# NVIDIA/tacotron2

Hardware: NVIDIA B200
Metric: mel frames/sec (B=64,T_text=150) (higher is better)
Workload: dtype f32 (split-fp16 tensor-core operands hi+lo, fp32 accumulate and state)

## Files before the change

### tacotron2_b200/_engine.py

```python
import contextlib
import ctypes as C
import threading

import torch

from . import _capi


def weight_table_spec(hp):
    E, K = hp.encoder_embedding_dim, hp.encoder_kernel_size
    s = [("embedding.weight", (hp.n_symbols, hp.symbols_embedding_dim))]

    def bn(p, c):
        return [(p + "weight", (c,)), (p + "bias", (c,)), (p + "running_mean", (c,)),
                (p + "running_var", (c,)), (p + "num_batches_tracked", ())]
    for i in range(hp.encoder_n_convolutions):
        p = "encoder.convolutions.%d." % i
        s += [(p + "0.conv.weight", (E, E, K)), (p + "0.conv.bias", (E,))] + bn(p + "1.", E)
    H = E // 2
    for suf in ("", "_reverse"):
        s += [("encoder.lstm.weight_ih_l0" + suf, (4 * H, E)), ("encoder.lstm.weight_hh_l0" + suf, (4 * H, H)),
              ("encoder.lstm.bias_ih_l0" + suf, (4 * H,)), ("encoder.lstm.bias_hh_l0" + suf, (4 * H,))]
    d = "decoder."
    nm = hp.n_mel_channels * hp.n_frames_per_step
    A, D, P = hp.attention_rnn_dim, hp.decoder_rnn_dim, hp.prenet_dim
    s += [(d + "prenet.layers.0.linear_layer.weight", (P, nm)), (d + "prenet.layers.1.linear_layer.weight", (P, P)),
          (d + "attention_rnn.weight_ih", (4 * A, P + E)), (d + "attention_rnn.weight_hh", (4 * A, A)),
          (d + "attention_rnn.bias_ih", (4 * A,)), (d + "attention_rnn.bias_hh", (4 * A,))]
    a = d + "attention_layer."
    s += [(a + "query_layer.linear_layer.weight", (hp.attention_dim, A)),
          (a + "memory_layer.linear_layer.weight", (hp.attention_dim, E)),
          (a + "v.linear_layer.weight", (1, hp.attention_dim)),
          (a + "location_layer.location_conv.conv.weight",
           (hp.attention_location_n_filters, 2, hp.attention_location_kernel_size)),
          (a + "location_layer.location_dense.linear_layer.weight", (hp.attention_dim, hp.attention_location_n_filters))]
    s += [(d + "decoder_rnn.weight_ih", (4 * D, A + E)), (d + "decoder_rnn.weight_hh", (4 * D, D)),
          (d + "decoder_rnn.bias_ih", (4 * D,)), (d + "decoder_rnn.bias_hh", (4 * D,)),
          (d + "linear_projection.linear_layer.weight", (nm, D + E)), (d + "linear_projection.linear_layer.bias", (nm,)),
          (d + "gate_layer.linear_layer.weight", (1, D + E)), (d + "gate_layer.linear_layer.bias", (1,))]
    PD, PK, n = hp.postnet_embedding_dim, hp.postnet_kernel_size, hp.postnet_n_convolutions
    for i in range(n):
        ci = hp.n_mel_channels if i == 0 else PD
        co = hp.n_mel_channels if i == n - 1 else PD
        p = "postnet.convolutions.%d." % i
        s += [(p + "0.conv.weight", (co, ci, PK)), (p + "0.conv.bias", (co,))] + bn(p + "1.", co)
    return s


_tls = threading.local()


@contextlib.contextmanager
def dropout_masks(prenet=None, att=None, dec=None, enc=None, post=None):
    prev = getattr(_tls, "masks", None)
    _tls.masks = dict(prenet=prenet, att=att, dec=dec, enc=enc, post=post)
    try:
        yield
    finally:
        _tls.masks = prev


def current_masks():
    return getattr(_tls, "masks", None) or dict(prenet=None, att=None, dec=None, enc=None, post=None)


_weights_generation = [0]


def bump_weights_generation():
    _weights_generation[0] += 1


def invalidate_weights():
    bump_weights_generation()


_seed_counter = [0]


def next_seed():
    _seed_counter[0] += 1
    return (torch.initial_seed() * 1000003 + _seed_counter[0]) & 0xFFFFFFFFFFFFFFFF


def _ptr(t):
    return C.c_void_p(t.data_ptr()) if t is not None else None


def _u8(mask, device):
    if mask is None:
        return None
    return mask.to(device=device, dtype=torch.uint8).contiguous()


class Engine:

    def __init__(self, hp):
        self.hp = hp
        self.spec = weight_table_spec(hp)
        self.handle = None
        self.key = None
        self.held = None
        self.device = None
        self._ws = {}
        self.impl = _capi.IMPL_AUTO

    def invalidate(self):
        self.key = None

    def ensure(self, named, force=False):
        dev = None
        for t in named.values():
            if t.is_cuda:
                dev = t.device
                break
        if dev is None:
            raise RuntimeError("tacotron2_b200: the model must live on a CUDA device (B200); there is no "
                               "CPU path -- call .cuda() first")
        key = (_weights_generation[0],) + tuple(
            (named[n].data_ptr(), named[n]._version, named[n].dtype) if n in named else None for n, _ in self.spec)
        if self.handle is not None and key == self.key and dev == self.device and not force:
            return
        L = _capi.lib()
        held, ptrs = [], (C.c_void_p * _capi.T2_NUM_WEIGHTS)()
        for i, (n, shape) in enumerate(self.spec):
            t = named.get(n)
            if n.endswith("num_batches_tracked"):
                ptrs[i] = None
                continue
            if t is None:
                t = torch.zeros(shape, device=dev, dtype=torch.float32)
                if n.endswith("running_var"):
                    t.fill_(1.0)
            else:
                if tuple(t.shape) != tuple(shape):
                    raise RuntimeError("tacotron2_b200: %s has shape %s, expected %s" % (n, tuple(t.shape), shape))
                t = t.detach()
                if t.dtype != torch.float32 or not t.is_contiguous():
                    t = t.float().contiguous()
            held.append(t)
            ptrs[i] = t.data_ptr()
        stream = C.c_void_p(torch.cuda.current_stream(dev).cuda_stream)
        with torch.cuda.device(dev):
            if self.handle is None or dev != self.device:
                self.close()
                hp = self.hp
                cfg = _capi.T2Config(
                    hp.n_mel_channels, hp.n_symbols, hp.symbols_embedding_dim, hp.encoder_kernel_size,
                    hp.encoder_n_convolutions, hp.encoder_embedding_dim, hp.attention_rnn_dim,
                    hp.decoder_rnn_dim, hp.prenet_dim, hp.attention_dim, hp.attention_location_n_filters,
                    hp.attention_location_kernel_size, hp.postnet_embedding_dim, hp.postnet_kernel_size,
                    hp.postnet_n_convolutions, hp.p_attention_dropout, hp.p_decoder_dropout, 1e-5)
                if hp.n_frames_per_step != 1:
                    raise RuntimeError("n_frames_per_step != 1 is not supported (hparams.py:56)")
                h = C.c_void_p()
                _capi.check(L.t2_model_create(C.byref(h), C.byref(cfg), ptrs, _capi.T2_NUM_WEIGHTS, stream))
                self.handle = h
            else:
                _capi.check(L.t2_model_refresh(self.handle, ptrs, _capi.T2_NUM_WEIGHTS, stream))
        self.key, self.held, self.device = key, held, dev

    def close(self):
        if self.handle is not None:
            _capi.lib().t2_model_destroy(self.handle)
            self.handle = None
            self.key = None

    def __del__(self):
        try:
            self.close()
        except Exception:
            pass

    def _workspace(self, tag, nbytes):
        t = self._ws.get(tag)
        if t is None or t.numel() < nbytes or t.device != self.device:
            t = torch.empty(int(nbytes), dtype=torch.uint8, device=self.device)
            self._ws[tag] = t
        return t

    def _stream(self):
        return C.c_void_p(torch.cuda.current_stream(self.device).cuda_stream)

    def encoder(self, text=None, embedded=None, lengths=None, training=False, keep=None, stash=None, seed=None):
        L = _capi.lib()
        src = text if text is not None else embedded
        B, T = int(src.shape[0]), int(src.shape[1])
        memory = torch.empty(B, T, self.hp.encoder_embedding_dim, device=self.device, dtype=torch.float32)
        ws = self._workspace("enc", L.t2_encoder_workspace_bytes(self.handle, B, T))
        a = _capi.T2EncoderArgs()
        if text is not None:
            text = text.to(device=self.device, dtype=torch.int64).contiguous()
            a.text = text.data_ptr()
        else:
            embedded = embedded.to(device=self.device, dtype=torch.float32).contiguous()
            a.embedded = embedded.data_ptr()
        len32 = None
        if lengths is not None:
            len32 = lengths.to(device=self.device, dtype=torch.int32).contiguous()
            a.lengths = len32.data_ptr()
        keep = _u8(keep, self.device)
        a.B, a.T, a.training = B, T, int(bool(training))
        a.keep = keep.data_ptr() if keep is not None else None
        a.seed = next_seed() if seed is None else seed
        a.memory, a.ws, a.ws_bytes = memory.data_ptr(), ws.data_ptr(), ws.numel()
        if stash is not None:
            a.stash, a.stash_bytes = stash.data_ptr(), stash.numel()
        with torch.cuda.device(self.device):
            _capi.check(L.t2_encoder_forward(self.handle, C.byref(a), self._stream()))
        return memory

    def stash_buffer(self, kind, *dims):
        n = getattr(_capi.lib(), "t2_%s_stash_bytes" % kind)(self.handle, *dims)
        return torch.empty(int(n), dtype=torch.uint8, device=self.device)

    def encoder_backward(self, text, embedded, lengths, training, keep, seed, stash, d_memory, want_d_embedded, named_grads):
        L = _capi.lib()
        B, T = int(d_memory.shape[0]), int(d_memory.shape[1])
        f32 = dict(device=self.device, dtype=torch.float32)
        a = _capi.T2EncoderBwdArgs()
        if text is not None:
            text = text.to(device=self.device, dtype=torch.int64).contiguous()
            a.text = text.data_ptr()
        else:
            embedded = embedded.to(**f32).contiguous()
            a.embedded = embedded.data_ptr()
        len32 = None
        if lengths is not None:
            len32 = lengths.to(device=self.device, dtype=torch.int32).contiguous()
            a.lengths = len32.data_ptr()
        keep = _u8(keep, self.device)
        a.B, a.T, a.training = B, T, int(bool(training))
        a.keep = keep.data_ptr() if keep is not None else None
        a.seed = seed
        a.stash, a.stash_bytes = stash.data_ptr(), stash.numel()
        d_memory = d_memory.to(**f32).contiguous()
        a.d_memory = d_memory.data_ptr()
        d_emb = torch.empty(B, T, self.hp.encoder_embedding_dim, **f32) if want_d_embedded else None
        a.d_embedded = d_emb.data_ptr() if d_emb is not None else None
        ptrs = self.grad_table(named_grads)
        a.grads, a.n_grads = ptrs, _capi.T2_NUM_WEIGHTS
        ws = self._workspace("enc_bwd", L.t2_encoder_backward_workspace_bytes(self.handle, B, T))
        a.ws, a.ws_bytes = ws.data_ptr(), ws.numel()
        with torch.cuda.device(self.device):
            _capi.check(L.t2_encoder_backward(self.handle, C.byref(a), self._stream()))
        return d_emb

    def postnet_backward(self, B, T, training, add_residual, keep, seed, stash, d_mel_post, named_grads, wgrad_lengths=None):
        L = _capi.lib()
        f32 = dict(device=self.device, dtype=torch.float32)
        a = _capi.T2PostnetBwdArgs()
        a.B, a.T, a.training, a.add_residual = B, T, int(bool(training)), int(bool(add_residual))
        if keep is not None and isinstance(keep, (list, tuple)):
            keep = torch.cat([k.to(torch.uint8).reshape(-1) for k in keep])
        keep = _u8(keep, self.device)
        a.keep = keep.data_ptr() if keep is not None else None
        a.seed = seed
        wl32 = None
        if wgrad_lengths is not None:
            wl32 = wgrad_lengths.to(device=self.device, dtype=torch.int32).contiguous()
            a.wgrad_lengths = wl32.data_ptr()
        a.stash, a.stash_bytes = stash.data_ptr(), stash.numel()
        d_mel_post = d_mel_post.to(**f32).contiguous()
        a.d_mel_post = d_mel_post.data_ptr()
        d_mel = torch.empty(B, T, self.hp.n_mel_channels, **f32)
        a.d_mel = d_mel.data_ptr()
        ptrs = self.grad_table(named_grads)
        a.grads, a.n_grads = ptrs, _capi.T2_NUM_WEIGHTS
        ws = self._workspace("post_bwd", L.t2_postnet_backward_workspace_bytes(self.handle, B, T))
        a.ws, a.ws_bytes = ws.data_ptr(), ws.numel()
        with torch.cuda.device(self.device):
            _capi.check(L.t2_postnet_backward(self.handle, C.byref(a), self._stream()))
        return d_mel

    def decoder(self, memory, mode, n_steps_cap, memory_lengths=None, teacher_prenet=None, training=False,
                prenet_keep=None, att_keep=None, dec_keep=None, gate_threshold=0.5,
                score_mask_value=-float("inf"), impl=None, stash=None, seed=None):
        L = _capi.lib()
        memory = memory.to(device=self.device, dtype=torch.float32).contiguous()
        B, T = int(memory.shape[0]), int(memory.shape[1])
        cap = int(n_steps_cap)
        mel = torch.zeros(B, cap, self.hp.n_mel_channels, device=self.device, dtype=torch.float32)
        gate = torch.zeros(B, cap, device=self.device, dtype=torch.float32)
        align = torch.zeros(B, cap, T, device=self.device, dtype=torch.float32)
        mel_lengths = torch.zeros(B, device=self.device, dtype=torch.int32)
        n_steps = torch.zeros(1, device=self.device, dtype=torch.int32)
        ws = self._workspace("dec", L.t2_decoder_workspace_bytes(self.handle, B, T, cap))
        a = _capi.T2DecoderArgs()
        a.mode, a.impl, a.training = mode, self.impl if impl is None else impl, int(bool(training))
        a.memory = memory.data_ptr()
        len32 = None
        if memory_lengths is not None:
            len32 = memory_lengths.to(device=self.device, dtype=torch.int32).contiguous()
            a.memory_lengths = len32.data_ptr()
        a.B, a.T_enc, a.n_steps_cap = B, T, cap
        if teacher_prenet is not None:
            teacher_prenet = teacher_prenet.contiguous()
            a.teacher_prenet = teacher_prenet.data_ptr()
        pk, ak, dk = _u8(prenet_keep, self.device), _u8(att_keep, self.device), _u8(dec_keep, self.device)
        a.prenet_keep = pk.data_ptr() if pk is not None else None
        a.att_keep = ak.data_ptr() if ak is not None else None
        a.dec_keep = dk.data_ptr() if dk is not None else None
        a.seed = next_seed() if seed is None else seed
        if stash is not None:
            a.stash, a.stash_bytes = stash.data_ptr(), stash.numel()
        a.gate_threshold = float(gate_threshold)
        a.score_mask_value = float(score_mask_value)
        a.mel, a.gate, a.align = mel.data_ptr(), gate.data_ptr(), align.data_ptr()
        a.mel_lengths, a.n_steps = mel_lengths.data_ptr(), n_steps.data_ptr()
        a.ws, a.ws_bytes = ws.data_ptr(), ws.numel()
        with torch.cuda.device(self.device):
            _capi.check(L.t2_decoder_run(self.handle, C.byref(a), self._stream()))
        self._last_decoder_args = (a, memory, len32, teacher_prenet, pk, ak, dk, ws, mel, gate, align, mel_lengths, n_steps)
        return mel, gate, align, mel_lengths, n_steps

    def decoder_profile(self):
        a = self._last_decoder_args[0]
        out = (C.c_int64 * 72)()
        _capi.check(_capi.lib().t2_decoder_profile(C.byref(a), out))
        names = ["E0 x2->att gemm", "E0 epilogue(ah)", "B1", "E1 ah->dec/att/q gemm", "B2", "attention", "B3",
                 "E2 ctx gemm", "E2 epilogue(dh)", "B4", "E3 dh gemm", "E3 epilogue(mel/x1)", "B5", "E4 x1 gemm+epi", "B6",
                 "att:im2col", "att:mma", "att:energies", "att:softmax", "att:context"]
        return {names[i]: [int(out[s * 24 + i]) for s in range(3)] for i in range(len(names))}

    def grad_table(self, named_grads):
        ptrs = (C.c_void_p * _capi.T2_NUM_WEIGHTS)()
        for i, (n, _) in enumerate(self.spec):
            t = named_grads.get(n)
            ptrs[i] = t.data_ptr() if t is not None else None
        return ptrs

    def decoder_stash(self, B, T_enc, T_mel):
        return self.stash_buffer("decoder", B, T_enc, T_mel)

    def decoder_backward(self, memory, memory_lengths, teacher_prenet, align, stash, seed, training, att_keep, dec_keep,
                         score_mask_value, d_mel, d_gate, d_align, named_grads):
        L = _capi.lib()
        B, Te = int(memory.shape[0]), int(memory.shape[1])
        T = int(align.shape[1])
        f32 = dict(device=self.device, dtype=torch.float32)
        d_memory = torch.empty(B, Te, self.hp.encoder_embedding_dim, **f32)
        d_prenet = torch.empty(T, B, self.hp.prenet_dim, **f32)
        ws = self._workspace("dec_bwd", L.t2_decoder_backward_workspace_bytes(self.handle, B, Te, T))
        a = _capi.T2DecoderBwdArgs()
        memory = memory.contiguous()
        a.memory = memory.data_ptr()
        len32 = None
        if memory_lengths is not None:
            len32 = memory_lengths.to(device=self.device, dtype=torch.int32).contiguous()
            a.memory_lengths = len32.data_ptr()
        a.B, a.T_enc, a.T_mel, a.training = B, Te, T, int(bool(training))
        a.teacher_prenet = teacher_prenet.data_ptr()
        ak, dk = _u8(att_keep, self.device), _u8(dec_keep, self.device)
        a.att_keep = ak.data_ptr() if ak is not None else None
        a.dec_keep = dk.data_ptr() if dk is not None else None
        a.seed, a.score_mask_value = seed, float(score_mask_value)
        a.align, a.stash, a.stash_bytes = align.data_ptr(), stash.data_ptr(), stash.numel()
        d_mel, d_gate = d_mel.to(**f32).contiguous(), d_gate.to(**f32).contiguous()
        a.d_mel, a.d_gate = d_mel.data_ptr(), d_gate.data_ptr()
        if d_align is not None:
            d_align = d_align.to(**f32).contiguous()
            a.d_align = d_align.data_ptr()
        a.d_memory, a.d_prenet = d_memory.data_ptr(), d_prenet.data_ptr()
        ptrs = self.grad_table(named_grads)
        a.grads, a.n_grads = ptrs, _capi.T2_NUM_WEIGHTS
        a.ws, a.ws_bytes = ws.data_ptr(), ws.numel()
        with torch.cuda.device(self.device):
            _capi.check(L.t2_decoder_backward(self.handle, C.byref(a), self._stream()))
        return d_memory, d_prenet

    def prenet_backward(self, frames, keep, seed, d_out, named_grads):
        L = _capi.lib()
        frames = frames.to(device=self.device, dtype=torch.float32).contiguous()
        M = int(frames.shape[0])
        d_out = d_out.contiguous()
        ws = self._workspace("pre_bwd", L.t2_prenet_backward_workspace_bytes(self.handle, M))
        keep = _u8(keep, self.device)
        a = _capi.T2PrenetBwdArgs()
        a.frames, a.M = frames.data_ptr(), M
        a.keep = keep.data_ptr() if keep is not None else None
        a.seed, a.d_out = seed, d_out.data_ptr()
        ptrs = self.grad_table(named_grads)
        a.grads, a.n_grads = ptrs, _capi.T2_NUM_WEIGHTS
        a.ws, a.ws_bytes = ws.data_ptr(), ws.numel()
        with torch.cuda.device(self.device):
            _capi.check(L.t2_prenet_backward(self.handle, C.byref(a), self._stream()))

    def prenet(self, frames, keep=None, seed=None):
        L = _capi.lib()
        frames = frames.to(device=self.device, dtype=torch.float32).contiguous()
        M = int(frames.shape[0])
        out = torch.empty(M, self.hp.prenet_dim, device=self.device, dtype=torch.float32)
        ws = self._workspace("pre", M * self.hp.prenet_dim * 4)
        keep = _u8(keep, self.device)
        with torch.cuda.device(self.device):
            _capi.check(L.t2_prenet_forward(self.handle, frames.data_ptr(), M,
                                            keep.data_ptr() if keep is not None else None,
                                            next_seed() if seed is None else seed,
                                            out.data_ptr(), ws.data_ptr(), ws.numel(), self._stream()))
        return out

    def postnet(self, mel_btc, lengths=None, add_residual=True, training=False, keep=None, stash=None, seed=None):
        L = _capi.lib()
        assert mel_btc.dtype == torch.float32 and mel_btc.stride(2) == 1 and mel_btc.stride(1) == mel_btc.shape[2]
        B, T = int(mel_btc.shape[0]), int(mel_btc.shape[1])
        out = torch.empty(B, self.hp.n_mel_channels, T, device=self.device, dtype=torch.float32)
        ws = self._workspace("post", L.t2_postnet_workspace_bytes(self.handle, B, T))
        a = _capi.T2PostnetArgs()
        a.mel, a.mel_batch_stride = mel_btc.data_ptr(), int(mel_btc.stride(0))
        len32 = None
        if lengths is not None:
            len32 = lengths.to(device=self.device, dtype=torch.int32).contiguous()
            a.lengths = len32.data_ptr()
        a.B, a.T, a.training = B, T, int(bool(training))
        if keep is not None and isinstance(keep, (list, tuple)):
            keep = torch.cat([k.to(torch.uint8).reshape(-1) for k in keep])
        keep = _u8(keep, self.device)
        a.keep = keep.data_ptr() if keep is not None else None
        a.seed = next_seed() if seed is None else seed
        a.add_residual = int(bool(add_residual))
        a.mel_post, a.ws, a.ws_bytes = out.data_ptr(), ws.data_ptr(), ws.numel()
        if stash is not None:
            a.stash, a.stash_bytes = stash.data_ptr(), stash.numel()
        with torch.cuda.device(self.device):
            _capi.check(L.t2_postnet_forward(self.handle, C.byref(a), self._stream()))
        return out

    def infer_host(self, text_host, max_steps, gate_threshold=0.5, impl=None, out_host=None):
        L = _capi.lib()
        B, T = int(text_host.shape[0]), int(text_host.shape[1])
        ws = self._workspace("e2e", L.t2_infer_workspace_bytes(self.handle, B, T, max_steps))
        if out_host is None:
            out_host = (torch.empty(B, self.hp.n_mel_channels, max_steps, dtype=torch.float32).pin_memory(),
                        torch.empty(B, dtype=torch.int32).pin_memory(), torch.empty(1, dtype=torch.int32).pin_memory())
        mel, lens, ns = out_host
        with torch.cuda.device(self.device):
            _capi.check(L.t2_infer_host(self.handle, text_host.data_ptr(), B, T, int(max_steps), float(gate_threshold),
                                        next_seed(), self.impl if impl is None else impl, mel.data_ptr(),
                                        lens.data_ptr(), ns.data_ptr(), ws.data_ptr(), ws.numel(), self._stream()))
        return mel, lens, ns
```

### tacotron2_b200/csrc/decoder.h

```cpp
#pragma once
#include "model.h"

namespace t2 {

constexpr int kMaxBatch = 1024;

struct DecoderCtrl {
  int all_done;
  int error;
  int pad_[2];
  unsigned int bar_count;
  unsigned int bar_gen;
  int pad2_[2];
  int done[kMaxBatch];
  long long prof[3][24];
  unsigned int x1_count; int pad3_[31];
  unsigned int x2_count; int pad4_[31];
  unsigned int ah_count[16]; int pad5_[16];
  unsigned int dh_count[16]; int pad6_[16];
};

struct DecoderWs {
  float* pm;
  char* state_begin; size_t state_bytes;
  float *ah, *ac, *dh, *dc;
  float* ctx;
  float *aw, *awc;
  float *x1, *x2;
  float* gates;
  float* proj;
  DecoderCtrl* ctrl;
  char* persistent; size_t persistent_bytes;
};

struct DecoderStash {
  float* ga = nullptr; float* gd = nullptr;
  float* ca = nullptr; float* ha = nullptr;
  float* cd = nullptr; float* hd = nullptr;
  float* ctx = nullptr;
};
inline size_t decoder_stash_bytes(int B, int T) {
  return ((size_t)2 * T * B * 4096 + (size_t)4 * (T + 1) * B * 1024 + (size_t)(T + 1) * B * 512) * sizeof(float);
}
inline void decoder_stash_carve(void* base, int B, int T, DecoderStash* s) {
  float* f = (float*)base;
  s->ga = f; f += (size_t)T * B * 4096;
  s->gd = f; f += (size_t)T * B * 4096;
  s->ca = f; f += (size_t)(T + 1) * B * 1024;
  s->ha = f; f += (size_t)(T + 1) * B * 1024;
  s->cd = f; f += (size_t)(T + 1) * B * 1024;
  s->hd = f; f += (size_t)(T + 1) * B * 1024;
  s->ctx = f;
}

size_t decoder_ws_bytes(int B, int T, int cap);
size_t persistent_ws_bytes(int B, int T, int cap);
int decoder_ws_carve(const T2DecoderArgs* a, DecoderWs* w);
int decoder_run_stepwise(T2Model* m, const T2DecoderArgs* a, cudaStream_t s);
int decoder_run_persistent(T2Model* m, const T2DecoderArgs* a, cudaStream_t s);
int decoder_backward(T2Model* m, const T2DecoderBwdArgs* a, cudaStream_t s);
size_t decoder_backward_ws_bytes(int B, int T_enc, int T_mel);
int prenet_backward(T2Model* m, const T2PrenetBwdArgs* a, cudaStream_t s);
bool persistent_supported(const T2Model* m, const T2DecoderArgs* a);

constexpr int kBwdGemmSplit = 4;
constexpr int kBwdImgBytes = 64 * 16384;
int bwd_gemm_prepare(T2Model* m, cudaStream_t s);
int bwd_gemm_run(T2Model* m, int which, const uint8_t* x_img, const float* inv_scale, float* P, int ldp, DecoderCtrl* ctrl,
                 cudaStream_t s);

}
```

### tacotron2_b200/csrc/decoder_persistent.cu

```cuda
#include <stdlib.h>
#include <string.h>

#include <vector>

#include "decoder.h"
#include "gemm_f32.cuh"
#include "umma.cuh"

namespace t2 {

namespace {

constexpr int kG = 128;
constexpr int kThreads = 512;
constexpr int kWarps = kThreads / 32;
constexpr int kStages = 4;
constexpr int kMaxStages = 5;
constexpr int kRows = 64;
constexpr int kXChunkBytes = 2 * kRows * kChunkK * 2;
constexpr int kColA = 0, kColD = 64, kColS = 128;
constexpr int kNA = 32, kND = 32, kNS = 16;
constexpr int kHiCols = 80;
constexpr int kColAtt = 160;
constexpr int kTmemCols = 512;
constexpr int kWStageMax = 2 * kHiCols * kChunkK * 2;
constexpr int kStageBytes = kXChunkBytes + kWStageMax;
constexpr int kNumEvents = 5;
constexpr int kPCols = 344;
constexpr int kQCta0 = 0, kQCtas = 16, kX2Cta0 = 16, kX2Ctas = 32, kPCta0 = 48, kPCtas = 43;
constexpr int kWeffBytes = kAtt * kChunkK * 2 * 2;
constexpr int kXchStride = 33;
constexpr unsigned long long kWatchdogCycles = 1ull << 32;

struct EventPlan {
  uint32_t w_off;
  uint32_t w_bytes;
  int32_t nrows;
  int32_t col0;
  int32_t ncons;
  int32_t n[3];
  int32_t chunks;
};
struct CtaPlan {
  EventPlan ev[kNumEvents];
};

struct BwdCta {
  EventPlan ep;
  int32_t chunk0, nchunks;
  int32_t col0, split;
};

struct PersistentPack {
  uint8_t* wimg = nullptr; size_t wimg_bytes = 0;
  CtaPlan* plans = nullptr;
  float* wp_all = nullptr;
  float* bias_p = nullptr;
  float* bias_a = nullptr;
  float* bias_d = nullptr;
  int32_t* rows = nullptr;
  float* weff = nullptr;
  uint8_t* weff_img = nullptr;
  uint8_t* bwd_wimg[2] = {nullptr, nullptr};
  struct BwdCta* bwd_plans[2] = {nullptr, nullptr};
};

__global__ void fuse_prenet_proj_kernel(const float* __restrict__ w1, const float* __restrict__ wp,
                                        const float* __restrict__ bp, float* __restrict__ out_w,
                                        float* __restrict__ out_b) {
  const int r = blockIdx.x;
  for (int c = threadIdx.x; c < kDRnn + kEnc; c += blockDim.x) {
    float s = 0.f;
    for (int k = 0; k < kMel; ++k) s = fmaf(w1[r * kMel + k], wp[(long)k * (kDRnn + kEnc) + c], s);
    out_w[(long)r * (kDRnn + kEnc) + c] = s;
  }
  if (threadIdx.x == 0) {
    float s = 0.f;
    for (int k = 0; k < kMel; ++k) s = fmaf(w1[r * kMel + k], bp[k], s);
    out_b[r] = s;
  }
}

__global__ void fuse_location_kernel(const float* __restrict__ wld, const float* __restrict__ wloc,
                                     float* __restrict__ weff) {
  const int d = blockIdx.x, kk = threadIdx.x;
  float s = 0.f;
  if (kk < 2 * kLocK) {
    const int ch = kk / kLocK, k = kk - ch * kLocK;
    for (int c = 0; c < kLocF; ++c) s = fmaf(wld[d * kLocF + c], wloc[(c * 2 + ch) * kLocK + k], s);
  }
  weff[d * kChunkK + kk] = s;
}

__global__ void pack_rows_image_kernel(const float* __restrict__ W, int N, int K, uint8_t* __restrict__ wimg) {
  const int chunk = blockIdx.x;
  __half* hi = reinterpret_cast<__half*>(wimg + (size_t)chunk * N * 256);
  __half* lo = hi + N * 64;
  for (int i = threadIdx.x; i < N * 64; i += blockDim.x) {
    const int r = i >> 6, k = i & 63;
    __half h, l;
    split_fp16(W[(long)r * K + chunk * 64 + k], h, l);
    const uint32_t e = img_elem_offset(r, k);
    hi[e] = h; lo[e] = l;
  }
}

__global__ void pack_consumer_kernel(const float* __restrict__ src, int ld, int kcol0,
                                     const int32_t* __restrict__ rows_tab, const CtaPlan* __restrict__ plans,
                                     int ev, int cons, uint8_t* __restrict__ wimg) {
  const int cta = blockIdx.y, chunk = blockIdx.x;
  const EventPlan& ep = plans[cta].ev[ev];
  if (cons >= ep.ncons) return;
  const int n = ep.n[cons];
  int roff = 0;
  for (int i = 0; i < cons; ++i) roff += 2 * ep.n[i];
  __half* img = reinterpret_cast<__half*>(wimg + ep.w_off + (size_t)chunk * ep.w_bytes);
  for (int i = threadIdx.x; i < n * 64; i += blockDim.x) {
    const int r = i >> 6, k = i & 63;
    const int srow = rows_tab[cta * 32 + r];
    const float v = srow >= 0 ? src[(long)srow * ld + kcol0 + chunk * 64 + k] : 0.f;
    __half h, l;
    split_fp16(v, h, l);
    img[img_elem_offset(roff + r, k)] = h;
    img[img_elem_offset(roff + n + r, k)] = l;
  }
}

__global__ void pack_lstm_bias_kernel(const float* __restrict__ b_sum, float* __restrict__ out) {
  const int i = blockIdx.x * blockDim.x + threadIdx.x;
  if (i >= kG * 32) return;
  const int cta = i >> 5, col = i & 31, ul = col >> 2, g = col & 3;
  out[i] = b_sum[g * 1024 + cta * 8 + ul];
}

__global__ void rows_to_image_kernel(const float* __restrict__ src, long ld, int n_rows, int K,
                                     long src_block_stride, uint8_t* __restrict__ dst, long dst_block_stride) {
  const float* s = src + (long)blockIdx.y * src_block_stride;
  uint8_t* d = dst + (long)blockIdx.y * dst_block_stride;
  const int chunk = blockIdx.x;
  __half* hi = reinterpret_cast<__half*>(d + (long)chunk * kXChunkBytes);
  __half* lo = hi + kRows * kChunkK;
  for (int i = threadIdx.x; i < kRows * kChunkK; i += blockDim.x) {
    const int r = i >> 6, k = i & 63;
    const int kk = chunk * kChunkK + k;
    const float v = (r < n_rows && kk < K) ? s[(long)r * ld + kk] : 0.f;
    __half h, l;
    split_fp16(v, h, l);
    const uint32_t e = img_elem_offset(r, k);
    hi[e] = h; lo[e] = l;
  }
}

__device__ __forceinline__ void watchdog_trap(DecoderCtrl* ctrl, int code) {
  if (ctrl) ctrl->error = code;
  __threadfence_system();
  __trap();
}

__device__ __forceinline__ void mbar_wait(uint64_t* bar, uint32_t parity, DecoderCtrl* ctrl, int code) {
  if (ptx::mbar_try_wait(bar, parity)) return;
  const unsigned long long t0 = clock64();
  while (!ptx::mbar_try_wait(bar, parity)) {
    if (clock64() - t0 > kWatchdogCycles) watchdog_trap(ctrl, code);
  }
}

__device__ __forceinline__ void arrive_release(unsigned int* cnt) {
  asm volatile("fence.acq_rel.gpu;" ::: "memory");
  asm volatile("red.relaxed.gpu.global.add.u32 [%0], 1;" ::"l"(cnt) : "memory");
}
__device__ __forceinline__ void poll_acquire(unsigned int* cnt, unsigned int target, DecoderCtrl* ctrl, int code) {
  const unsigned long long t0 = clock64();
  while (true) {
    unsigned int c;
    asm volatile("ld.relaxed.gpu.global.u32 %0, [%1];" : "=r"(c) : "l"(cnt) : "memory");
    if ((int)(c - target) >= 0) break;
    if (clock64() - t0 > kWatchdogCycles) watchdog_trap(ctrl, code);
  }
  asm volatile("fence.acq_rel.gpu;" ::: "memory");
}

__device__ __forceinline__ void grid_barrier(DecoderCtrl* ctrl, unsigned int& target, uint32_t cs, uint32_t rank) {
  ptx::fence_proxy_async();
  if (cs > 1) {
    __threadfence();
    ptx::cluster_sync_all();
    target += gridDim.x / cs;
    if (rank == 0 && threadIdx.x == 0) {
      asm volatile("red.release.gpu.global.add.u32 [%0], 1;" ::"l"(&ctrl->bar_count) : "memory");
      const unsigned long long t0 = clock64();
      while (true) {
        unsigned int c;
        asm volatile("ld.acquire.gpu.global.u32 %0, [%1];" : "=r"(c) : "l"(&ctrl->bar_count) : "memory");
        if ((int)(c - target) >= 0) break;
        if (clock64() - t0 > kWatchdogCycles) watchdog_trap(ctrl, 100);
      }
      __threadfence();
    }
    ptx::cluster_sync_all();
    ptx::fence_proxy_async();
    return;
  }
  __syncthreads();
  target += gridDim.x;
  if (threadIdx.x == 0) {
    arrive_release(&ctrl->bar_count);
    poll_acquire(&ctrl->bar_count, target, ctrl, 100);
  }
  __syncthreads();
  ptx::fence_proxy_async();
}

__device__ __forceinline__ void grid_arrive(DecoderCtrl* ctrl, unsigned int& target) {
  ptx::fence_proxy_async();
  __syncthreads();
  target += gridDim.x;
  if (threadIdx.x == 0) {
    arrive_release(&ctrl->bar_count);
  }
}
__device__ __forceinline__ void grid_wait(DecoderCtrl* ctrl, unsigned int target) {
  if (threadIdx.x == 0) {
    poll_acquire(&ctrl->bar_count, target, ctrl, 101);
  }
  __syncthreads();
  ptx::fence_proxy_async();
}

constexpr unsigned int kStopFlag = 1u << 24;
__device__ __forceinline__ void signal_counter(unsigned int* cnt, unsigned int inc) {
  ptx::fence_proxy_async();
  __syncthreads();
  if (threadIdx.x == 0) {
    asm volatile("fence.acq_rel.gpu;" ::: "memory");
    asm volatile("red.relaxed.gpu.global.add.u32 [%0], %1;" ::"l"(cnt), "r"(inc) : "memory");
  }
}
__device__ __forceinline__ bool wait_counter(unsigned int* cnt, unsigned int target, int* s_flag, DecoderCtrl* ctrl, int code) {
  if (threadIdx.x == 0) {
    const unsigned long long t0 = clock64();
    unsigned int c;
    while (true) {
      asm volatile("ld.relaxed.gpu.global.u32 %0, [%1];" : "=r"(c) : "l"(cnt) : "memory");
      if ((c & (kStopFlag - 1u)) >= target) break;
      if (clock64() - t0 > kWatchdogCycles) watchdog_trap(ctrl, code);
    }
    asm volatile("fence.acq_rel.gpu;" ::: "memory");
    *s_flag = (int)(c >> 24);
  }
  __syncthreads();
  ptx::fence_proxy_async();
  return *s_flag != 0;
}

__device__ __forceinline__ float sigmoid_exact(float x) { return 1.f / (1.f + expf(-x)); }
__device__ __forceinline__ float sigmoid_fast(float x) { return __fdividef(1.f, 1.f + __expf(-x)); }
__device__ __forceinline__ float tanh_fast(float x) { return 2.f * sigmoid_fast(2.f * x) - 1.f; }
__device__ __forceinline__ float warp_sum_f(float v) {
#pragma unroll
  for (int o = 16; o > 0; o >>= 1) v += __shfl_xor_sync(0xffffffffu, v, o);
  return v;
}
__device__ __forceinline__ float warp_max_f(float v) {
#pragma unroll
  for (int o = 16; o > 0; o >>= 1) v = fmaxf(v, __shfl_xor_sync(0xffffffffu, v, o));
  return v;
}

struct Ring {
  uint8_t* stage0;
  __device__ __forceinline__ uint8_t* stage(uint32_t s) const { return stage0 + s * kStageBytes; }
  uint64_t* full;
  uint64_t* empty;
  uint64_t* acc;
  uint32_t p_stage, p_phase;
  uint32_t c_stage, c_phase;
  uint32_t acc_phase;
  uint64_t pol_x, pol_w;
  uint32_t cs, rank;
  uint32_t pre;
  uint32_t ns;
};

__device__ __forceinline__ void prefetch_weights(Ring& rg, const EventPlan& nx, const uint8_t* w_img,
                                                 DecoderCtrl* ctrl) {
  uint32_t s = rg.p_stage, ph = rg.p_phase;
  const uint32_t n = min(rg.ns, (uint32_t)nx.chunks);
  for (uint32_t i = 0; i < n; ++i) {
    mbar_wait(&rg.empty[s], ph ^ 1, ctrl, 205);
    ptx::mbar_arrive_expect_tx(&rg.full[s], kXChunkBytes + nx.w_bytes);
    ptx::bulk_g2s_hint(rg.stage(s) + kXChunkBytes, w_img + nx.w_off + (size_t)i * nx.w_bytes, nx.w_bytes,
                       &rg.full[s], rg.pol_w);
    if (++s == rg.ns) { s = 0; ph ^= 1; }
  }
  rg.pre = n;
}

__device__ __forceinline__ void run_event(Ring& rg, const EventPlan& ep, const uint8_t* x_img,
                                          const uint8_t* w_img, int chunks, uint32_t tmem_base,
                                          DecoderCtrl* ctrl, const EventPlan* next,
                                          const unsigned int* ready = nullptr, unsigned int ready_target = 0) {
  const int warp = threadIdx.x >> 5, lane = threadIdx.x & 31;
  if (ep.nrows == 0) {
    if (threadIdx.x == 0 && next != nullptr && next->nrows != 0 && rg.pre == 0) prefetch_weights(rg, *next, w_img, ctrl);
    return;
  }
  if (warp == 0) {
    if (lane == 0) {
      int nready = ready ? 0 : chunks;
      for (int i = 0; i < chunks; ++i) {
        uint8_t* st = rg.stage(rg.p_stage);
        if ((uint32_t)i >= rg.pre) {
          mbar_wait(&rg.empty[rg.p_stage], rg.p_phase ^ 1, ctrl, 200);
          ptx::mbar_arrive_expect_tx(&rg.full[rg.p_stage], kXChunkBytes + ep.w_bytes);
          ptx::bulk_g2s_hint(st + kXChunkBytes, w_img + ep.w_off + (size_t)i * ep.w_bytes, ep.w_bytes,
                             &rg.full[rg.p_stage], rg.pol_w);
        }
        if (i >= nready) {
          const unsigned long long t0 = clock64();
          while (true) {
            uint32_t c[16];
#pragma unroll
            for (int j = 0; j < 16; j += 4)
              asm volatile("ld.relaxed.gpu.global.v4.u32 {%0,%1,%2,%3}, [%4];"
                           : "=r"(c[j]), "=r"(c[j + 1]), "=r"(c[j + 2]), "=r"(c[j + 3]) : "l"(ready + j) : "memory");
            uint32_t mask = 0;
#pragma unroll
            for (int j = 0; j < 16; ++j) mask |= ((int)(c[j] - ready_target) >= 0 ? 1u : 0u) << j;
            const int run = __ffs((int)~(mask >> i)) - 1;
            if (run > 0) { nready = min(chunks, i + run); break; }
            if (clock64() - t0 > kWatchdogCycles) watchdog_trap(ctrl, 206);
          }
          asm volatile("fence.acq_rel.gpu;" ::: "memory");
          ptx::fence_proxy_async();
        }
        if (rg.cs == 1) {
          ptx::bulk_g2s_hint(st, x_img + (size_t)i * kXChunkBytes, kXChunkBytes, &rg.full[rg.p_stage], rg.pol_x);
        } else {
          const uint32_t slice = kXChunkBytes / rg.cs;
          ptx::bulk_g2s_mc_hint(st + rg.rank * slice, x_img + (size_t)i * kXChunkBytes + rg.rank * slice, slice,
                                &rg.full[rg.p_stage], (uint16_t)((1u << rg.cs) - 1u), rg.pol_x);
        }
        if (++rg.p_stage == rg.ns) { rg.p_stage = 0; rg.p_phase ^= 1; }
      }
      rg.pre = 0;
      if (next != nullptr && next->nrows != 0) prefetch_weights(rg, *next, w_img, ctrl);
    }
    __syncwarp();
  } else if (warp == 1) {
    if (lane == 0) {
      const uint32_t idesc = ptx::make_idesc_f16(128, 2u * (uint32_t)ep.nrows);
      const uint32_t d = tmem_base + (uint32_t)ep.col0;
      for (int i = 0; i < chunks; ++i) {
        mbar_wait(&rg.full[rg.c_stage], rg.c_phase, ctrl, 201);
        ptx::tc_fence_after();
        const uint32_t xs = ptx::smem_u32(rg.stage(rg.c_stage));
        const uint32_t ws = xs + kXChunkBytes;
#pragma unroll
        for (int kk = 0; kk < kChunkK / 16; ++kk) {
          const uint64_t a = ptx::make_sw128_desc(xs + kk * 32);
          const uint64_t b = ptx::make_sw128_desc(ws + kk * 32);
          ptx::umma_f16(d, a, b, idesc, 1u);
        }
        if (rg.cs == 1) ptx::umma_commit(&rg.empty[rg.c_stage]);
        else ptx::umma_commit_mc(&rg.empty[rg.c_stage], (uint16_t)((1u << rg.cs) - 1u));
        if (++rg.c_stage == rg.ns) { rg.c_stage = 0; rg.c_phase ^= 1; }
      }
      ptx::umma_commit(rg.acc);
    }
    __syncwarp();
  }
  mbar_wait(rg.acc, rg.acc_phase, ctrl, 202);
  rg.acc_phase ^= 1;
  ptx::tc_fence_after();
}

__device__ __forceinline__ uint32_t philox_keep8(uint64_t seed, uint32_t site, uint64_t idx0, float pdrop) {
  uint32_t bits = 0;
  uint64_t blk_cur = ~0ull;
  uint32_t o[4] = {0, 0, 0, 0};
#pragma unroll
  for (int i = 0; i < 8; ++i) {
    const uint64_t idx = idx0 + i, blk = idx >> 2;
    if (blk != blk_cur) {
      philox4x32_10((uint32_t)blk, (uint32_t)(blk >> 32), site, 0x7ac07201u, (uint32_t)seed, (uint32_t)(seed >> 32), o);
      blk_cur = blk;
    }
    const float u = (float)(o[idx & 3] >> 8) * (1.0f / 16777216.0f);
    bits |= (u >= pdrop ? 1u : 0u) << i;
  }
  return bits;
}

__device__ __forceinline__ void acc_take8(uint32_t t_lane, int base, int n, int col, float* s) {
  float a[8], b[8];
  ptx::tmem_ld8(t_lane + base + col, a);
  ptx::tmem_ld8(t_lane + base + n + col, b);
#pragma unroll
  for (int i = 0; i < 8; ++i) s[i] = a[i] + b[i];
  ptx::tmem_zero8(t_lane + base + col);
  ptx::tmem_zero8(t_lane + base + n + col);
  ptx::tmem_wait_st();
}

__device__ __forceinline__ void stash_lstm(float* gates, float* cs, float* hs, int t, int Btot, int b, int unit0,
                                           const float (&sg)[4][2], const float (&c)[2], const float (&h)[2]) {
  float* gp = gates + ((long)t * Btot + b) * (4 * kARnn) + unit0;
#pragma unroll
  for (int g = 0; g < 4; ++g) *reinterpret_cast<float2*>(gp + g * kARnn) = make_float2(sg[g][0], sg[g][1]);
  const long o = ((long)(t + 1) * Btot + b) * kARnn + unit0;
  *reinterpret_cast<float2*>(cs + o) = make_float2(c[0], c[1]);
  *reinterpret_cast<float2*>(hs + o) = make_float2(h[0], h[1]);
}

struct KParams {
  const CtaPlan* plans;
  const uint8_t* wimg;
  const float* bias_a; const float* bias_d; const float* bias_p;
  const uint8_t* weff_img; const float* w_v;
  float l2_pin_frac;
  const float* memory; const float* pm; const int32_t* mem_len;
  const uint8_t* prenet_keep; const uint8_t* att_keep; const uint8_t* dec_keep;
  uint8_t* x2_img; uint8_t* ah_img; uint8_t* ctx_img; uint8_t* dh_img; uint8_t* x1_img;
  const uint8_t* teacher_x2_img;
  float* q;
  float* mel; float* gate; float* align; int32_t* mel_lengths; int32_t* n_steps;
  DecoderCtrl* ctrl;
  int B, T, cap, infer, training, cluster, hier_barrier;
  int nstages;
  int chunk_ready;
  int b0, Btot;
  float gate_threshold, score_mask_value, p_att, p_dec;
  uint64_t seed;
  DecoderStash st;
};

__device__ __forceinline__ void store_split2(uint8_t* img, int row, int k, float v0, float v1) {
  const int chunk = k >> 6, kc = k & 63;
  __half h0, l0, h1, l1;
  split_fp16(v0, h0, l0);
  split_fp16(v1, h1, l1);
  __half* hi = reinterpret_cast<__half*>(img + (size_t)chunk * kXChunkBytes);
  __half* lo = hi + kRows * kChunkK;
  const uint32_t e = img_elem_offset(row, kc);
  *reinterpret_cast<__half2*>(hi + e) = __halves2half2(h0, h1);
  *reinterpret_cast<__half2*>(lo + e) = __halves2half2(l0, l1);
}

__global__ void __launch_bounds__(kThreads, 1) decoder_persistent_kernel(const KParams p) {
  extern __shared__ __align__(1024) uint8_t smem_raw[];
  const int tid = threadIdx.x, warp = tid >> 5, lane = tid & 31;
  const int cta = blockIdx.x;
  const int T = p.T, TP = T + kLocK - 1;
  const int ntiles = (T + 127) >> 7;

  uint8_t* sp = smem_raw;
  Ring rg;
  rg.ns = (uint32_t)p.nstages;
  rg.stage0 = sp; sp += p.nstages * kStageBytes;
  uint8_t* s_weff = sp; sp += kWeffBytes;
  uint64_t* bars = reinterpret_cast<uint64_t*>(sp); sp += 16 * sizeof(uint64_t);
  rg.full = bars; rg.empty = bars + kMaxStages; rg.acc = bars + 2 * kMaxStages;
  uint32_t* tmem_slot = reinterpret_cast<uint32_t*>(sp); sp += 16;
  int* s_live = reinterpret_cast<int*>(sp); sp += 16;
  int* s_flag = s_live + 1;
  float* s_bias_a = reinterpret_cast<float*>(sp); sp += 32 * 4;
  float* s_bias_d = reinterpret_cast<float*>(sp); sp += 32 * 4;
  float* s_v = reinterpret_cast<float*>(sp); sp += kAtt * 4;
  float* s_q = reinterpret_cast<float*>(sp); sp += kAtt * 4;
  float* s_red = reinterpret_cast<float*>(sp); sp += 32 * 4;
  uint32_t* s_mask = reinterpret_cast<uint32_t*>(sp); sp += kRows * 4;
  float* s_bias_p = reinterpret_cast<float*>(sp); sp += 8 * 4;
  long long* s_prof = reinterpret_cast<long long*>(sp); sp += 24 * 8;
  float* s_pad0 = reinterpret_cast<float*>(sp); sp += ((TP + 3) & ~3) * 4;
  float* s_pad1 = reinterpret_cast<float*>(sp); sp += ((TP + 3) & ~3) * 4;
  float* s_xch = reinterpret_cast<float*>(sp);
  float* s_e = reinterpret_cast<float*>(sp);
  float* s_ep = s_e + ntiles * 128;
  (void)s_red;

  rg.p_stage = rg.p_phase = rg.c_stage = rg.c_phase = rg.acc_phase = 0;
  rg.cs = p.cluster; rg.rank = p.cluster > 1 ? ptx::cluster_ctarank() : 0;
  rg.pre = 0;

  if (tid == 0) {
    for (int s = 0; s < p.nstages; ++s) { ptx::mbar_init(&rg.full[s], 1); ptx::mbar_init(&rg.empty[s], rg.cs); }
    ptx::mbar_init(rg.acc, 1);
    ptx::fence_barrier_init();
  }
  if (warp == 2) ptx::tmem_alloc<kTmemCols>(tmem_slot);
  for (int i = tid; i < 32; i += kThreads) { s_bias_a[i] = p.bias_a[cta * 32 + i]; s_bias_d[i] = p.bias_d[cta * 32 + i]; }
  for (int i = tid; i < kWeffBytes / 16; i += kThreads)
    reinterpret_cast<uint4*>(s_weff)[i] = reinterpret_cast<const uint4*>(p.weff_img)[i];
  {
    uint64_t pol;
    asm volatile("createpolicy.fractional.L2::evict_last.L2::evict_first.b64 %0, %1;" : "=l"(pol) : "f"(p.l2_pin_frac));
    rg.pol_w = pol;
    rg.pol_x = ptx::policy_evict_last();
  }
  for (int i = tid; i < kAtt; i += kThreads) s_v[i] = p.w_v[i];
  if (tid < 8) s_bias_p[tid] = (cta >= kPCta0 && cta < kPCta0 + kPCtas) ? p.bias_p[(cta - kPCta0) * 8 + tid] : 0.f;
  for (int i = tid; i < TP; i += kThreads) { s_pad0[i] = 0.f; s_pad1[i] = 0.f; }
  ptx::fence_proxy_async();
  ptx::tc_fence_before();
  __syncthreads();
  if (p.cluster > 1) ptx::cluster_sync_all();
  ptx::tc_fence_after();
  const uint32_t tmem_base = *tmem_slot;

  const CtaPlan& plan = p.plans[cta];
  DecoderCtrl* ctrl = p.ctrl;
  unsigned int bar_target = 0;
  const uint32_t bar_cs = p.hier_barrier ? rg.cs : 1;
  const int quad = warp & 3, cg = warp >> 2;
  const int row = (quad & 1) * 32 + lane;
  const bool is_lo = quad >= 2;
  const bool erow = !is_lo && row < p.B;
  const uint32_t t_lane = tmem_base + ((uint32_t)(quad * 32) << 16);
  float c_att[2] = {0.f, 0.f}, c_dec[2] = {0.f, 0.f};
  const bool has_q = cta >= kQCta0 && cta < kQCta0 + kQCtas;
  const bool has_x2 = cta >= kX2Cta0 && cta < kX2Cta0 + kX2Ctas;
  const bool has_p = cta >= kPCta0 && cta < kPCta0 + kPCtas;
  const int halfk = (kLocK - 1) / 2;
  for (int c = cg * 40; c < cg * 40 + 40; c += 8) ptx::tmem_zero8(t_lane + c);
  ptx::tmem_wait_st();
  ptx::tc_fence_before();
  __syncthreads();
  const int prof_slot = cta == 0 ? 0 : (cta == 60 ? 1 : (cta == 100 ? 2 : -1));
  long long prof_last = clock64();
  if (tid < 24) s_prof[tid] = 0;
#define T2_PROF(ph)                                                        \
  do {                                                                     \
    if (prof_slot >= 0 && tid == 0) {                                      \
      const long long now_ = clock64();                                    \
      s_prof[ph] += now_ - prof_last;    \
      prof_last = now_;                                                    \
    }                                                                      \
  } while (0)
#define T2_TAKE_GATES(colbase, n_, g)                                                        \
  do {                                                                                   \
    acc_take8(t_lane, (colbase), (n_), cg * 8, g);                                       \
    if (is_lo) {                                                                         \
      _Pragma("unroll") for (int i_ = 0; i_ < 8; ++i_) s_xch[row * kXchStride + cg * 8 + i_] = g[i_]; \
    }                                                                                    \
    ptx::tc_fence_before();                                                              \
    __syncthreads();                                                                     \
    if (!is_lo) {                                                                        \
      _Pragma("unroll") for (int i_ = 0; i_ < 8; ++i_) g[i_] += s_xch[row * kXchStride + cg * 8 + i_]; \
    }                                                                                    \
  } while (0)

  auto x2_epilogue = [&]() {
    float g[8];
    if (cg == 0) acc_take8(t_lane, kColS, kNS, 0, g);
    if (cg == 0 && is_lo) {
#pragma unroll
      for (int i = 0; i < 8; ++i) s_xch[row * kXchStride + i] = g[i];
    }
    ptx::tc_fence_before();
    __syncthreads();
    if (cg == 0 && erow) {
      const int col0 = (cta - kX2Cta0) * 8;
      float r[8];
      const uint32_t bits = s_mask[row];
#pragma unroll
      for (int j = 0; j < 8; ++j)
        r[j] = ((bits >> j) & 1u) ? fmaxf(g[j] + s_xch[row * kXchStride + j], 0.f) * 2.f : 0.f;
#pragma unroll
      for (int j = 0; j < 8; j += 2) store_split2(p.x2_img, row, col0 + j, r[j], r[j + 1]);
    }
  };

  int t = 0;
  for (; t < p.cap; ++t) {
    {
      const uint8_t* x2 = p.infer ? p.x2_img : p.teacher_x2_img + (size_t)t * 4 * kXChunkBytes;
      run_event(rg, plan.ev[0], x2, p.wimg, 4, tmem_base, ctrl, &plan.ev[1]);
      T2_PROF(0);
      float g[8];
      T2_TAKE_GATES(kColA, kNA, g);
      if (erow) {
        float hv[2], sg[4][2];
#pragma unroll
        for (int u = 0; u < 2; ++u) {
          const float* b = s_bias_a + (cg * 2 + u) * 4;
          const float gi = sigmoid_fast(g[u * 4 + 0] + b[0]);
          const float gf = sigmoid_fast(g[u * 4 + 1] + b[1]);
          const float gg = tanh_fast(g[u * 4 + 2] + b[2]);
          const float go = sigmoid_fast(g[u * 4 + 3] + b[3]);
          c_att[u] = gf * c_att[u] + gi * gg;
          float h = go * tanh_fast(c_att[u]);
          if (p.training) {
            const int unit = cta * 8 + cg * 2 + u;
            const long idx = (long)(p.b0 + row) * kARnn + unit;
            const bool keep = p.att_keep ? p.att_keep[(long)t * p.Btot * kARnn + idx] != 0
                                         : philox_keep(p.seed, t * 4 + 2, idx, p.p_att);
            h = keep ? h * (1.f / (1.f - p.p_att)) : 0.f;
          }
          hv[u] = h;
          sg[0][u] = gi; sg[1][u] = gf; sg[2][u] = gg; sg[3][u] = go;
        }
        store_split2(p.ah_img, row, cta * 8 + cg * 2, hv[0], hv[1]);
        if (p.st.ga) stash_lstm(p.st.ga, p.st.ca, p.st.ha, t, p.Btot, p.b0 + row, cta * 8 + cg * 2, sg, c_att, hv);
      }
      T2_PROF(1);
      if (p.chunk_ready) signal_counter(&ctrl->ah_count[cta >> 3], 1u);
      else grid_barrier(ctrl, bar_target, bar_cs, rg.rank);
      T2_PROF(2);
    }
    {
      if (p.infer && is_lo && cg == 0 && row < p.B && t + 1 < p.cap && (has_p || has_x2)) {
        uint32_t bits = 0;
        if (has_x2) {
          const int col0 = (cta - kX2Cta0) * 8;
          if (p.prenet_keep) {
            const uint8_t* kp = p.prenet_keep + ((long)(t + 1) * 2 + 1) * p.Btot * kPre + (long)(p.b0 + row) * kPre + col0;
            for (int j = 0; j < 8; ++j) bits |= (kp[j] != 0 ? 1u : 0u) << j;
          } else {
            bits = philox_keep8(p.seed, (t + 1) * 4 + 1, (uint64_t)(p.b0 + row) * kPre + col0, 0.5f);
          }
        } else {
          const int pc0 = (cta - kPCta0) * 8;
          for (int j = 0; j < 8; ++j) {
            const int col = pc0 + j - (kMel + 1);
            if (col < 0 || col >= kPre) continue;
            const long idx = (long)(p.b0 + row) * kPre + col;
            const bool keep = p.prenet_keep ? p.prenet_keep[((long)(t + 1) * 2 + 0) * p.Btot * kPre + idx] != 0
                                            : philox_keep(p.seed, (t + 1) * 4 + 0, idx, 0.5f);
            bits |= (keep ? 1u : 0u) << j;
          }
        }
        s_mask[row] = bits;
      }
      run_event(rg, plan.ev[1], p.ah_img, p.wimg, 16, tmem_base, ctrl, nullptr,
                p.chunk_ready ? ctrl->ah_count : nullptr, 8u * (unsigned int)(t + 1));
      if (has_q) {
        float g[8];
        if (cg == 0) acc_take8(t_lane, kColS, kNS, 0, g);
        if (cg == 0 && is_lo) {
#pragma unroll
          for (int i = 0; i < 8; ++i) s_xch[row * kXchStride + i] = g[i];
        }
        ptx::tc_fence_before();
        __syncthreads();
        if (cg == 0 && erow) {
#pragma unroll
          for (int j = 0; j < 8; ++j) p.q[row * kAtt + (cta - kQCta0) * 8 + j] = g[j] + s_xch[row * kXchStride + j];
        }
      }
      T2_PROF(3);
    }
    const bool att_cta = (cta & 63) < p.B;
    const int att_b = cta & 63, ahalf = cta >> 6;
    uint8_t* aimg = rg.stage0;
    const int att_rounds = (T + 255) >> 8;
    const int img_plane = att_rounds > 1 ? 32768 : max(4096, ((T + 15) & ~15) * 128);
    const int img_bytes = 2 * img_plane;
    const int smem_rows = min(T, (p.nstages * kStageBytes - img_bytes) / (kEnc / 2 * 4));
    auto att_im2col_mma_tr = [&](int r0) {
      const int jbase = r0 * 256, cnt = min(T - jbase, 256), npad = (cnt + 15) & ~15;
      for (int item = tid; item < npad * 8; item += kThreads) {
        const int jj = item >> 3, g8 = item & 7, j = jbase + jj;
        __align__(16) __half hh[8];
        __align__(16) __half ll[8];
#pragma unroll
        for (int e = 0; e < 8; ++e) {
          const int kk = g8 * 8 + e;
          float v = 0.f;
          if (jj < cnt && kk < 2 * kLocK) v = kk < kLocK ? s_pad0[j + kk] : s_pad1[j + kk - kLocK];
          split_fp16(v, hh[e], ll[e]);
        }
        uint8_t* dst = aimg + (jj >> 3) * 1024 + (jj & 7) * 128 + ((g8 ^ (jj & 7)) * 16);
        *reinterpret_cast<uint4*>(dst) = *reinterpret_cast<const uint4*>(hh);
        *reinterpret_cast<uint4*>(dst + img_plane) = *reinterpret_cast<const uint4*>(ll);
      }
      ptx::fence_proxy_async();
      __syncthreads();
      if (warp == 1) {
        if (lane == 0) {
          ptx::tc_fence_after();
          const uint32_t ws = ptx::smem_u32(s_weff), ps = ptx::smem_u32(aimg);
          const uint32_t idesc = ptx::make_idesc_f16(128, (uint32_t)npad);
          const uint32_t d = tmem_base + kColAtt;
#pragma unroll
          for (int kk = 0; kk < kChunkK / 16; ++kk) {
            const uint64_t w_hi = ptx::make_sw128_desc(ws + kk * 32);
            const uint64_t w_lo = ptx::make_sw128_desc(ws + 16384 + kk * 32);
            const uint64_t p_hi = ptx::make_sw128_desc(ps + kk * 32);
            const uint64_t p_lo = ptx::make_sw128_desc(ps + (uint32_t)img_plane + kk * 32);
            ptx::umma_f16(d, w_hi, p_hi, idesc, kk > 0 ? 1u : 0u);
            ptx::umma_f16(d, w_lo, p_hi, idesc, 1u);
            ptx::umma_f16(d, w_hi, p_lo, idesc, 1u);
          }
          ptx::umma_commit(rg.acc);
        }
        __syncwarp();
      }
    };
    auto stage_memory_rows = [&](int j0, int j1) {
      const uint32_t sbase = ptx::smem_u32(rg.stage0) + (uint32_t)img_bytes;
      const float* msrc = p.memory + (long)att_b * T * kEnc + ahalf * (kEnc / 2);
      for (int i = j0 * 64 + tid; i < j1 * 64; i += kThreads) {
        const int j = i >> 6, c4 = i & 63;
        asm volatile("cp.async.cg.shared.global [%0], [%1], 16;" ::"r"(sbase + (uint32_t)i * 16u),
                     "l"(msrc + (long)j * kEnc + c4 * 4)
                     : "memory");
      }
      asm volatile("cp.async.commit_group;" ::: "memory");
    };
    grid_arrive(ctrl, bar_target);
    const int adim = quad * 32 + lane;
    float pm_next[8];
    auto load_pm = [&](const float* pmr, int j0, int cnt) {
#pragma unroll
      for (int e = 0; e < 8; ++e) pm_next[e] = (j0 + e < cnt) ? __ldg(pmr + (long)(j0 + e) * kAtt) : 0.f;
    };
    if (att_cta) {
      att_im2col_mma_tr(0);
      stage_memory_rows(0, smem_rows);
      load_pm(p.pm + (long)att_b * T * kAtt + adim, cg * 8, min(T, 256));
    }
    T2_PROF(15);
    grid_wait(ctrl, bar_target);
    T2_PROF(4);
    if (att_cta) {
      const int b = att_b;
      for (int i = tid; i < kAtt; i += kThreads) s_q[i] = __ldcg(&p.q[b * kAtt + i]);
      __syncthreads();
      {
        const int eN = ntiles * 128;
        const float qd = s_q[adim], vd = s_v[adim];
        const int nrounds = att_rounds;
        for (int r0 = 0; r0 < nrounds; ++r0) {
          const int jbase = r0 * 256, cnt = min(T - jbase, 256), nch = (((cnt + 15) & ~15) >> 3);
          if (r0 > 0) att_im2col_mma_tr(r0);
          mbar_wait(rg.acc, rg.acc_phase, ctrl, 203);
          rg.acc_phase ^= 1;
          ptx::tc_fence_after();
          T2_PROF(16);
          const float* pmr = p.pm + ((long)b * T + jbase) * kAtt + adim;
          if (r0 > 0) load_pm(pmr, cg * 8, cnt);
#pragma unroll 1
          for (int c = cg; c < nch; c += 4) {
            const int j0 = c * 8;
            float pm8[8];
#pragma unroll
            for (int e = 0; e < 8; ++e) pm8[e] = pm_next[e];
            if (c + 4 < nch) load_pm(pmr, j0 + 32, cnt);
            float g[8], sv[8];
            ptx::tmem_ld8(t_lane + kColAtt + j0, g);
#pragma unroll
            for (int e = 0; e < 8; ++e) sv[e] = vd * tanh_fast(qd + g[e] + pm8[e]);
            float r4[4], r2[2], r1;
            {
              const bool up = (lane & 16) != 0;
#pragma unroll
              for (int e = 0; e < 4; ++e) {
                const float send = up ? sv[e] : sv[e + 4], keep = up ? sv[e + 4] : sv[e];
                r4[e] = keep + __shfl_xor_sync(0xffffffffu, send, 16);
              }
            }
            {
              const bool up = (lane & 8) != 0;
#pragma unroll
              for (int e = 0; e < 2; ++e) {
                const float send = up ? r4[e] : r4[e + 2], keep = up ? r4[e + 2] : r4[e];
                r2[e] = keep + __shfl_xor_sync(0xffffffffu, send, 8);
              }
            }
            {
              const bool up = (lane & 4) != 0;
              const float send = up ? r2[0] : r2[1], keep = up ? r2[1] : r2[0];
              r1 = keep + __shfl_xor_sync(0xffffffffu, send, 4);
            }
            r1 += __shfl_xor_sync(0xffffffffu, r1, 2);
            r1 += __shfl_xor_sync(0xffffffffu, r1, 1);
            const int jj = j0 + ((lane >> 4) & 1) * 4 + ((lane >> 3) & 1) * 2 + ((lane >> 2) & 1);
            if ((lane & 3) == 0 && jj < cnt) s_ep[quad * eN + jbase + jj] = r1;
          }
          ptx::tc_fence_before();
          __syncthreads();
          T2_PROF(17);
        }
      }
      const int len = p.mem_len ? p.mem_len[b] : T;
      const int eN = ntiles * 128;
      for (int j = tid; j < T; j += kThreads)
        s_ep[j] = (j < len) ? (s_ep[j] + s_ep[eN + j]) + (s_ep[2 * eN + j] + s_ep[3 * eN + j]) : p.score_mask_value;
      __syncthreads();
      float mx = -INFINITY;
      for (int j = lane; j < T; j += 32) mx = fmaxf(mx, s_ep[j]);
      mx = warp_max_f(mx);
      float sum = 0.f;
      for (int j = lane; j < T; j += 32) sum += expf(s_ep[j] - mx);
      sum = warp_sum_f(sum);
      const float inv = 1.f / sum;
      for (int j = tid; j < T; j += kThreads) {
        const float a = expf(s_ep[j] - mx) * inv;
        s_e[j] = a;
        s_pad0[halfk + j] = a;
        s_pad1[halfk + j] += a;
        if (ahalf == 0) p.align[((long)b * p.cap + t) * T + j] = a;
      }
      asm volatile("cp.async.wait_group 0;" ::: "memory");
      __syncthreads();
      T2_PROF(18);
      {
        const int c4 = tid & 63, jg = tid >> 6;
        const float4* ms = reinterpret_cast<const float4*>(rg.stage0 + img_bytes);
        float4 acc = make_float4(0.f, 0.f, 0.f, 0.f);
#pragma unroll 4
        for (int j = jg; j < smem_rows; j += 8) {
          const float4 m = ms[j * 64 + c4];
          const float a = s_e[j];
          acc.x = fmaf(a, m.x, acc.x); acc.y = fmaf(a, m.y, acc.y); acc.z = fmaf(a, m.z, acc.z); acc.w = fmaf(a, m.w, acc.w);
        }
        const float* mp = p.memory + (long)b * T * kEnc + ahalf * (kEnc / 2) + c4 * 4;
        for (int j = smem_rows + jg; j < T; j += 8) {
          const float4 m = __ldg(reinterpret_cast<const float4*>(mp + (long)j * kEnc));
          const float a = s_e[j];
          acc.x = fmaf(a, m.x, acc.x); acc.y = fmaf(a, m.y, acc.y); acc.z = fmaf(a, m.z, acc.z); acc.w = fmaf(a, m.w, acc.w);
        }
        __syncthreads();
        float* scr = reinterpret_cast<float*>(rg.stage0);
        *reinterpret_cast<float4*>(scr + jg * (kEnc / 2) + c4 * 4) = acc;
        __syncthreads();
        if (tid < kEnc / 4) {
          const int col = tid * 2;
          float v0 = 0.f, v1 = 0.f;
#pragma unroll
          for (int g = 0; g < 8; ++g) { v0 += scr[g * (kEnc / 2) + col]; v1 += scr[g * (kEnc / 2) + col + 1]; }
          store_split2(p.ctx_img, b, ahalf * (kEnc / 2) + col, v0, v1);
          if (p.st.ga)
            *reinterpret_cast<float2*>(p.st.ctx + ((long)(t + 1) * p.Btot + p.b0 + b) * kEnc + ahalf * (kEnc / 2) + col) =
                make_float2(v0, v1);
        }
      }
      T2_PROF(19);
    }
    T2_PROF(5);
    grid_barrier(ctrl, bar_target, bar_cs, rg.rank);
    T2_PROF(6);
    {
      run_event(rg, plan.ev[2], p.ctx_img, p.wimg, 8, tmem_base, ctrl, &plan.ev[3]);
      T2_PROF(7);
      float g[8];
      T2_TAKE_GATES(kColD, kND, g);
      if (erow) {
        float hv[2], sg[4][2];
#pragma unroll
        for (int u = 0; u < 2; ++u) {
          const float* b = s_bias_d + (cg * 2 + u) * 4;
          const float gi = sigmoid_fast(g[u * 4 + 0] + b[0]);
          const float gf = sigmoid_fast(g[u * 4 + 1] + b[1]);
          const float gg = tanh_fast(g[u * 4 + 2] + b[2]);
          const float go = sigmoid_fast(g[u * 4 + 3] + b[3]);
          c_dec[u] = gf * c_dec[u] + gi * gg;
          float h = go * tanh_fast(c_dec[u]);
          if (p.training) {
            const int unit = cta * 8 + cg * 2 + u;
            const long idx = (long)(p.b0 + row) * kDRnn + unit;
            const bool keep = p.dec_keep ? p.dec_keep[(long)t * p.Btot * kDRnn + idx] != 0
                                         : philox_keep(p.seed, t * 4 + 3, idx, p.p_dec);
            h = keep ? h * (1.f / (1.f - p.p_dec)) : 0.f;
          }
          hv[u] = h;
          sg[0][u] = gi; sg[1][u] = gf; sg[2][u] = gg; sg[3][u] = go;
        }
        store_split2(p.dh_img, row, cta * 8 + cg * 2, hv[0], hv[1]);
        if (p.st.ga) stash_lstm(p.st.gd, p.st.cd, p.st.hd, t, p.Btot, p.b0 + row, cta * 8 + cg * 2, sg, c_dec, hv);
      }
      T2_PROF(8);
      if (p.chunk_ready) signal_counter(&ctrl->dh_count[cta >> 3], 1u);
      else grid_barrier(ctrl, bar_target, bar_cs, rg.rank);
      T2_PROF(9);
    }
    {
      run_event(rg, plan.ev[3], p.dh_img, p.wimg, 16, tmem_base, ctrl,
                (!p.infer && t + 1 < p.cap) ? &plan.ev[0] : nullptr,
                p.chunk_ready ? ctrl->dh_count : nullptr, 8u * (unsigned int)(t + 1));
      T2_PROF(10);
      if (tid == 0) *s_live = 0;
      float g[8];
      if (has_p && cg == 0) acc_take8(t_lane, kColS, kNS, 0, g);
      if (has_p && cg == 0 && is_lo) {
#pragma unroll
        for (int i = 0; i < 8; ++i) s_xch[row * kXchStride + i] = g[i];
      }
      ptx::tc_fence_before();
      __syncthreads();
      if (has_p && cg == 0 && erow) {
        const int pc0 = (cta - kPCta0) * 8;
#pragma unroll
        for (int j = 0; j < 8; ++j) {
          const int pc = pc0 + j;
          const float v = g[j] + s_xch[row * kXchStride + j] + s_bias_p[j];
          if (pc < kMel) {
            p.mel[((long)row * p.cap + t) * kMel + pc] = v;
          } else if (pc == kMel) {
            p.gate[(long)row * p.cap + t] = v;
            if (p.infer) {
              int done = ctrl->done[row];
              if (!done && sigmoid_exact(v) > p.gate_threshold) {
                done = 1; ctrl->done[row] = 1; p.mel_lengths[row] = t + 1;
              }
              if (!done) atomicAdd(s_live, 1);
            }
          } else if (pc < kMel + 1 + kPre) {
            const int col = pc - (kMel + 1);
            float r = fmaxf(v, 0.f);
            if (p.infer && t + 1 < p.cap) r = ((s_mask[row] >> j) & 1u) ? r * 2.f : 0.f;
            if (p.infer) {
              __half h, l;
              split_fp16(r, h, l);
              __half* hi = reinterpret_cast<__half*>(p.x1_img + (size_t)(col >> 6) * kXChunkBytes);
              __half* lo = hi + kRows * kChunkK;
              const uint32_t e = img_elem_offset(row, col & 63);
              hi[e] = h; lo[e] = l;
            }
          }
        }
      }
      __syncthreads();
      const bool gate_cta = has_p && (cta - kPCta0) * 8 <= kMel && (cta - kPCta0) * 8 + 8 > kMel;
      if (gate_cta && tid == 0) atomicMax(p.n_steps, t + 1);
      T2_PROF(11);
      if (!p.infer) continue;
      bool stop = t + 1 == p.cap;
      if (has_p) signal_counter(&ctrl->x1_count, 1u + ((gate_cta && *s_live == 0) ? kStopFlag : 0u));
      if (has_x2) {
        stop |= wait_counter(&ctrl->x1_count, (unsigned int)(kPCtas * (t + 1)), s_flag, ctrl, 102);
        if (!stop) {
          run_event(rg, plan.ev[4], p.x1_img, p.wimg, 4, tmem_base, ctrl, nullptr);
          x2_epilogue();
        }
        signal_counter(&ctrl->x2_count, 1u + (stop ? kStopFlag : 0u));
      }
      T2_PROF(12);
      stop |= wait_counter(&ctrl->x2_count, (unsigned int)(kX2Ctas * (t + 1)), s_flag, ctrl, 103);
      T2_PROF(14);
      if (stop) { ++t; break; }
    }
  }
  if (prof_slot >= 0 && tid == 0)
    for (int i = 0; i < 24; ++i) ctrl->prof[prof_slot][i] = s_prof[i];
  if (cta == 0) {
    __syncthreads();
    const int ns = p.infer ? t : p.cap;
    for (int b = tid; b < p.B; b += kThreads)
      if (!p.infer || !__ldcg(&ctrl->done[b])) p.mel_lengths[b] = ns;
    if (tid == 0) atomicMax(p.n_steps, ns);
  }
  if (p.cluster > 1) {
    if (tid == 0)
      for (int s = 0; s < p.nstages; ++s) {
        mbar_wait(&rg.empty[rg.p_stage], rg.p_phase ^ 1, ctrl, 204);
        if (++rg.p_stage == rg.ns) { rg.p_stage = 0; rg.p_phase ^= 1; }
      }
    __syncthreads();
    ptx::cluster_sync_all();
  }
  ptx::tc_fence_before();
  __syncthreads();
  if (warp == 2) ptx::tmem_dealloc<kTmemCols>(tmem_base);
}

}

static size_t persistent_smem_bytes(int T, int nstages) {
  const int TP = T + kLocK - 1;
  const int ntiles = (T + 127) / 128;
  const size_t xch = (size_t)kRows * kXchStride * 4, att = (size_t)5 * ntiles * 128 * 4;
  return (size_t)nstages * kStageBytes + kWeffBytes + 16 * 8 + 16 + 16 + 2 * 32 * 4 + kAtt * 4 + kAtt * 4 + 32 * 4 +
         kRows * 4 + 32 + 24 * 8 + 2 * (size_t)((TP + 3) & ~3) * 4 + (xch > att ? xch : att) + 1024;
}
constexpr size_t kSmemLimit = 227 * 1024;
static int persistent_stages(int T) {
  int want = 4;
  const char* e = getenv("T2_STAGES");
  if (e && atoi(e) >= 3 && atoi(e) <= kMaxStages) want = atoi(e);
  while (want > 4 && persistent_smem_bytes(T, want) > kSmemLimit) --want;
  return want;
}

size_t persistent_ws_bytes(int B, int T, int cap) {
  (void)B; (void)T;
  return (size_t)(4 + 16 + 8 + 16 + 4) * kXChunkBytes + (size_t)kRows * kAtt * 4 + 1024 +
         (size_t)cap * 4 * kXChunkBytes;
}

bool persistent_supported(const T2Model* m, const T2DecoderArgs* a) {
  if (!m->pk) return false;
  if (m->sm_count < kG) return false;
  if (persistent_smem_bytes(a->T_enc, 4) > kSmemLimit) return false;
  return true;
}

int persistent_pack_create(T2Model* m, cudaStream_t s) {
  PersistentPack* pk = (PersistentPack*)m->pk;
  if (!pk) { pk = new PersistentPack(); m->pk = pk; }
  const int kdc = kDRnn + kEnc;
  std::vector<CtaPlan> plans(kG);
  size_t off = 0;
  for (int c = 0; c < kG; ++c) {
    const bool hq = c >= kQCta0 && c < kQCta0 + kQCtas, hx = c >= kX2Cta0 && c < kX2Cta0 + kX2Ctas,
               hp = c >= kPCta0 && c < kPCta0 + kPCtas;
    CtaPlan& pl = plans[c];
    memset(&pl, 0, sizeof(pl));
    auto set = [&](int ev, int chunks, int col0, std::initializer_list<int> ns) {
      EventPlan& e = pl.ev[ev];
      e.ncons = 0; e.nrows = 0; e.col0 = col0;
      for (int n : ns) { e.n[e.ncons++] = n; e.nrows += n; }
      e.w_bytes = (uint32_t)e.nrows * 256;
      e.w_off = (uint32_t)off;
      e.chunks = chunks;
      off += (size_t)chunks * e.w_bytes;
    };
    set(0, 4, kColA, {32});
    if (hq) set(1, 16, kColA, {32, 32, 16}); else set(1, 16, kColA, {32, 32});
    if (hp) set(2, 8, kColA, {32, 32, 16}); else set(2, 8, kColA, {32, 32});
    if (hp) set(3, 16, kColD, {32, 16}); else set(3, 16, kColD, {32});
    if (hx) set(4, 4, kColS, {16}); else { pl.ev[4].w_off = (uint32_t)off; }
  }
  if (off >= (size_t)4 << 30) return fail(T2_ERR_INVALID, "W image too large");
  if (!pk->wimg) {
    pk->wimg_bytes = off + 1024;
    T2_CUDA(cudaMalloc((void**)&pk->wimg, pk->wimg_bytes));
    T2_CUDA(cudaMalloc((void**)&pk->plans, sizeof(CtaPlan) * kG));
    T2_CUDA(cudaMalloc((void**)&pk->wp_all, (size_t)kPCols * kdc * 4));
    T2_CUDA(cudaMalloc((void**)&pk->bias_p, (size_t)kPCols * 4));
    T2_CUDA(cudaMalloc((void**)&pk->bias_a, (size_t)kG * 32 * 4));
    T2_CUDA(cudaMalloc((void**)&pk->bias_d, (size_t)kG * 32 * 4));
    T2_CUDA(cudaMalloc((void**)&pk->rows, (size_t)4 * kG * 32 * 4));
    T2_CUDA(cudaMalloc((void**)&pk->weff, (size_t)kAtt * kChunkK * 4));
    T2_CUDA(cudaMalloc((void**)&pk->weff_img, (size_t)kWeffBytes));
  }
  fuse_location_kernel<<<kAtt, kChunkK, 0, s>>>(m->w[W_ATT_LOC_DENSE], m->w[W_ATT_LOC_CONV], pk->weff);
  T2_LAUNCH_CHECK();
  pack_rows_image_kernel<<<1, 256, 0, s>>>(pk->weff, kAtt, kChunkK, pk->weff_img);
  T2_LAUNCH_CHECK();
  T2_CUDA(cudaMemcpyAsync(pk->plans, plans.data(), sizeof(CtaPlan) * kG, cudaMemcpyHostToDevice, s));
  T2_CUDA(cudaStreamSynchronize(s));
  T2_CUDA(cudaMemsetAsync(pk->wp_all, 0, (size_t)kPCols * kdc * 4, s));
  T2_CUDA(cudaMemsetAsync(pk->bias_p, 0, (size_t)kPCols * 4, s));
  T2_CUDA(cudaMemcpyAsync(pk->wp_all, m->projgate_w, (size_t)(kMel + 1) * kdc * 4, cudaMemcpyDeviceToDevice, s));
  T2_CUDA(cudaMemcpyAsync(pk->bias_p, m->projgate_b, (size_t)(kMel + 1) * 4, cudaMemcpyDeviceToDevice, s));
  fuse_prenet_proj_kernel<<<kPre, 256, 0, s>>>(m->w[W_PRENET0], m->w[W_PROJ_W], m->w[W_PROJ_B],
                                               pk->wp_all + (size_t)(kMel + 1) * kdc, pk->bias_p + kMel + 1);
  T2_LAUNCH_CHECK();
  pack_lstm_bias_kernel<<<(kG * 32 + 255) / 256, 256, 0, s>>>(m->arnn_b, pk->bias_a);
  T2_LAUNCH_CHECK();
  pack_lstm_bias_kernel<<<(kG * 32 + 255) / 256, 256, 0, s>>>(m->drnn_b, pk->bias_d);
  T2_LAUNCH_CHECK();
  std::vector<int32_t> rows((size_t)4 * kG * 32, -1);
  for (int c = 0; c < kG; ++c) {
    for (int col = 0; col < 32; ++col) rows[(0 * kG + c) * 32 + col] = (col & 3) * 1024 + c * 8 + (col >> 2);
    if (c >= kQCta0 && c < kQCta0 + kQCtas) for (int j = 0; j < 8; ++j) rows[(1 * kG + c) * 32 + j] = (c - kQCta0) * 8 + j;
    if (c >= kPCta0 && c < kPCta0 + kPCtas) for (int j = 0; j < 8; ++j) rows[(2 * kG + c) * 32 + j] = (c - kPCta0) * 8 + j;
    if (c >= kX2Cta0 && c < kX2Cta0 + kX2Ctas) for (int j = 0; j < 8; ++j) rows[(3 * kG + c) * 32 + j] = (c - kX2Cta0) * 8 + j;
  }
  T2_CUDA(cudaMemcpyAsync(pk->rows, rows.data(), rows.size() * 4, cudaMemcpyHostToDevice, s));
  T2_CUDA(cudaStreamSynchronize(s));
  const int32_t* r_lstm = pk->rows; const int32_t* r_q = pk->rows + kG * 32;
  const int32_t* r_p = pk->rows + 2 * kG * 32; const int32_t* r_x2 = pk->rows + 3 * kG * 32;
  auto pack = [&](const float* src, int ld, int kcol0, int chunks, const int32_t* rt, int ev, int cons) -> int {
    pack_consumer_kernel<<<dim3(chunks, kG), 256, 0, s>>>(src, ld, kcol0, rt, pk->plans, ev, cons, pk->wimg);
    T2_LAUNCH_CHECK();
    return T2_OK;
  };
  T2_TRY(pack(m->w[W_ARNN_WIH], kPre + kEnc, 0, 4, r_lstm, 0, 0));
  T2_TRY(pack(m->w[W_ARNN_WHH], kARnn, 0, 16, r_lstm, 1, 0));
  T2_TRY(pack(m->w[W_DRNN_WIH], kdc, 0, 16, r_lstm, 1, 1));
  T2_TRY(pack(m->w[W_ATT_QUERY], kARnn, 0, 16, r_q, 1, 2));
  T2_TRY(pack(m->w[W_ARNN_WIH], kPre + kEnc, kPre, 8, r_lstm, 2, 0));
  T2_TRY(pack(m->w[W_DRNN_WIH], kdc, kARnn, 8, r_lstm, 2, 1));
  T2_TRY(pack(pk->wp_all, kdc, kDRnn, 8, r_p, 2, 2));
  T2_TRY(pack(m->w[W_DRNN_WHH], kDRnn, 0, 16, r_lstm, 3, 0));
  T2_TRY(pack(pk->wp_all, kdc, 0, 16, r_p, 3, 1));
  T2_TRY(pack(m->w[W_PRENET1], kPre, 0, 4, r_x2, 4, 0));
  return T2_OK;
}

void persistent_pack_destroy(T2Model* m) {
  PersistentPack* pk = (PersistentPack*)m->pk;
  if (!pk) return;
  cudaFree(pk->wimg); cudaFree(pk->plans); cudaFree(pk->wp_all); cudaFree(pk->bias_p);
  cudaFree(pk->bias_a); cudaFree(pk->bias_d); cudaFree(pk->rows); cudaFree(pk->weff); cudaFree(pk->weff_img);
  for (int i = 0; i < 2; ++i) { cudaFree(pk->bwd_wimg[i]); cudaFree(pk->bwd_plans[i]); }
  delete pk;
  m->pk = nullptr;
}

static int run_persistent_slice(T2Model* m, const T2DecoderArgs* a, cudaStream_t s, int b0, int nb);

int decoder_run_persistent(T2Model* m, const T2DecoderArgs* a, cudaStream_t s) {
  T2_CUDA(cudaMemsetAsync(a->n_steps, 0, sizeof(int32_t), s));
  for (int b0 = 0; b0 < a->B; b0 += kRows) {
    const int nb = a->B - b0 < kRows ? a->B - b0 : kRows;
    T2_TRY(run_persistent_slice(m, a, s, b0, nb));
  }
  return T2_OK;
}

static int run_persistent_slice(T2Model* m, const T2DecoderArgs* a, cudaStream_t s, int b0, int nb) {
  PersistentPack* pk = (PersistentPack*)m->pk;
  const int B = nb, T = a->T_enc, cap = a->n_steps_cap;
  DecoderWs w;
  T2_TRY(decoder_ws_carve(a, &w));
  T2_CUDA(cudaMemsetAsync(w.ctrl, 0, sizeof(DecoderCtrl), s));
  T2_CUDA(cudaMemsetAsync(w.persistent, 0, (size_t)(4 + 16 + 8 + 16 + 4) * kXChunkBytes + (size_t)kRows * kAtt * 4, s));
  {
    GemmArgs g;
    g.seg[0] = {a->memory + (size_t)b0 * T * kEnc, kEnc, m->w[W_ATT_MEMORY], kEnc, kEnc};
    g.M = B * T; g.N = kAtt; g.C = w.pm; g.ldc = kAtt;
    T2_TRY(gemm_f32(g, s));
  }
  KParams p;
  memset(&p, 0, sizeof(p));
  uint8_t* img = (uint8_t*)w.persistent;
  p.x2_img = img; img += 4 * kXChunkBytes;
  p.ah_img = img; img += 16 * kXChunkBytes;
  p.ctx_img = img; img += 8 * kXChunkBytes;
  p.dh_img = img; img += 16 * kXChunkBytes;
  p.x1_img = img; img += 4 * kXChunkBytes;
  p.q = (float*)img;
  p.plans = pk->plans; p.wimg = pk->wimg; p.bias_a = pk->bias_a; p.bias_d = pk->bias_d; p.bias_p = pk->bias_p;
  p.weff_img = pk->weff_img; p.w_v = m->w[W_ATT_V];
  {
    const char* e = getenv("T2_L2_PIN_FRAC");
    p.l2_pin_frac = e ? (float)atof(e) : 0.5f;
  }
  p.memory = a->memory + (size_t)b0 * T * kEnc; p.pm = w.pm;
  p.mem_len = a->memory_lengths ? a->memory_lengths + b0 : nullptr;
  p.prenet_keep = a->prenet_keep; p.att_keep = a->att_keep; p.dec_keep = a->dec_keep;
  p.mel = a->mel + (size_t)b0 * cap * kMel; p.gate = a->gate + (size_t)b0 * cap; p.align = a->align + (size_t)b0 * cap * T;
  p.mel_lengths = a->mel_lengths + b0; p.n_steps = a->n_steps;
  p.ctrl = w.ctrl;
  p.b0 = b0; p.Btot = a->B;
  p.B = B; p.T = T; p.cap = cap; p.infer = a->mode == T2_MODE_INFER; p.training = a->training;
  p.gate_threshold = a->gate_threshold; p.score_mask_value = a->score_mask_value;
  p.p_att = m->cfg.p_attention_dropout; p.p_dec = m->cfg.p_decoder_dropout; p.seed = a->seed;
  if (a->stash) {
    if (p.infer) return fail(T2_ERR_INVALID, "the training stash needs T2_MODE_TEACHER");
    if (a->stash_bytes < decoder_stash_bytes(a->B, cap)) return fail(T2_ERR_WORKSPACE, "decoder stash too small");
    decoder_stash_carve(a->stash, a->B, cap, &p.st);
    if (b0 == 0) {
      float* z[5] = {p.st.ca, p.st.ha, p.st.cd, p.st.hd, p.st.ctx};
      for (int i = 0; i < 5; ++i)
        T2_CUDA(cudaMemsetAsync(z[i], 0, (size_t)a->B * (i < 4 ? kARnn : kEnc) * sizeof(float), s));
    }
  }
  if (!p.infer) {
    uint8_t* timg = (uint8_t*)p.q + (size_t)kRows * kAtt * 4;
    timg = (uint8_t*)(((uintptr_t)timg + 1023) & ~(uintptr_t)1023);
    rows_to_image_kernel<<<dim3(4, cap), 256, 0, s>>>(a->teacher_prenet + (size_t)b0 * kPre, kPre, B, kPre, (long)a->B * kPre, timg,
                                                      (long)4 * kXChunkBytes);
    T2_LAUNCH_CHECK();
    p.teacher_x2_img = timg;
  }
  p.nstages = persistent_stages(T);
  {
  }
  {
    const char* e = getenv("T2_CHUNK_READY");
    p.chunk_ready = (e && !strcmp(e, "0")) ? 0 : 1;
  }
  const size_t smem = persistent_smem_bytes(T, p.nstages);
  T2_CUDA(cudaFuncSetAttribute(decoder_persistent_kernel, cudaFuncAttributeMaxDynamicSharedMemorySize, (int)smem));
  T2_CUDA(cudaFuncSetAttribute(decoder_persistent_kernel, cudaFuncAttributeNonPortableClusterSizeAllowed, 1));
  int want = 1;
  {
    const char* e = getenv("T2_CLUSTER");
    if (e) want = atoi(e);
    if (want != 1 && want != 2 && want != 4 && want != 8) want = 1;
  }
  {
    p.hier_barrier = 0;
  }
  cudaLaunchConfig_t cfg;
  memset(&cfg, 0, sizeof(cfg));
  cfg.gridDim = dim3(kG); cfg.blockDim = dim3(kThreads); cfg.dynamicSmemBytes = smem; cfg.stream = s;
  cudaLaunchAttribute attrs[2];
  for (p.cluster = want; p.cluster > 1; p.cluster >>= 1) {
    attrs[0].id = cudaLaunchAttributeClusterDimension;
    attrs[0].val.clusterDim.x = p.cluster; attrs[0].val.clusterDim.y = 1; attrs[0].val.clusterDim.z = 1;
    cfg.attrs = attrs; cfg.numAttrs = 1;
    int max_clusters = 0;
    if (cudaOccupancyMaxActiveClusters(&max_clusters, decoder_persistent_kernel, &cfg) == cudaSuccess &&
        max_clusters * p.cluster >= kG)
      break;
    (void)cudaGetLastError();
  }
  int na = 0;
  if (p.cluster > 1) {
    attrs[na].id = cudaLaunchAttributeClusterDimension;
    attrs[na].val.clusterDim.x = p.cluster; attrs[na].val.clusterDim.y = 1; attrs[na].val.clusterDim.z = 1; ++na;
  }
  attrs[na].id = cudaLaunchAttributeCooperative; attrs[na].val.cooperative = 1; ++na;
  cfg.attrs = attrs; cfg.numAttrs = na;
  cudaError_t le = cudaLaunchKernelEx(&cfg, decoder_persistent_kernel, p);
  if (le != cudaSuccess && p.cluster > 1) {
    (void)cudaGetLastError();
    cfg.numAttrs = 1;
    le = cudaLaunchKernelEx(&cfg, decoder_persistent_kernel, p);
  }
  if (le != cudaSuccess) return fail(T2_ERR_CUDA, "persistent decoder launch failed: %s", cudaGetErrorString(le));
  if (getenv("T2_VERBOSE")) fprintf(stderr, "[t2b200] persistent decoder: B=%d T_enc=%d cap=%d cluster=%d stages=%d chunk_ready=%d smem=%zu\n",
                                    B, T, cap, p.cluster, p.nstages, p.chunk_ready, smem);
  g_launch_count++;
  return T2_OK;
}

#ifdef T2_SELFTEST
namespace {
__global__ void __launch_bounds__(kThreads, 1)
selftest_kernel(const uint8_t* x_img, const uint8_t* w_img, EventPlan ep, int chunks, float* C, int N,
                DecoderCtrl* ctrl) {
  extern __shared__ __align__(1024) uint8_t smem_raw[];
  const int tid = threadIdx.x, warp = tid >> 5, lane = tid & 31;
  uint8_t* sp = smem_raw;
  Ring rg;
  rg.stage0 = sp; sp += kStages * kStageBytes;
  uint64_t* bars = reinterpret_cast<uint64_t*>(sp); sp += 16 * sizeof(uint64_t);
  rg.full = bars; rg.empty = bars + kStages; rg.acc = bars + 2 * kStages;
  uint32_t* tmem_slot = reinterpret_cast<uint32_t*>(sp); sp += 16;
  float* s_xch = reinterpret_cast<float*>(sp);
  rg.p_stage = rg.p_phase = rg.c_stage = rg.c_phase = rg.acc_phase = 0;
  rg.pol_x = rg.pol_w = ptx::policy_evict_last();
  rg.cs = 1; rg.rank = 0; rg.pre = 0; rg.ns = kStages;
  if (tid == 0) {
    for (int s = 0; s < kStages; ++s) { ptx::mbar_init(&rg.full[s], 1); ptx::mbar_init(&rg.empty[s], 1); }
    ptx::mbar_init(rg.acc, 1);
    ptx::fence_barrier_init();
  }
  if (warp == 2) ptx::tmem_alloc<kTmemCols>(tmem_slot);
  ptx::tc_fence_before();
  __syncthreads();
  ptx::tc_fence_after();
  const uint32_t tmem_base = *tmem_slot;
  const int quad = warp & 3, cg = warp >> 2;
  const uint32_t t_lane = tmem_base + ((uint32_t)(quad * 32) << 16);
  for (int c = cg * 40; c < cg * 40 + 40; c += 8) ptx::tmem_zero8(t_lane + c);
  ptx::tmem_wait_st();
  ptx::tc_fence_before();
  __syncthreads();
  run_event(rg, ep, x_img, w_img, chunks, tmem_base, ctrl, &ep);
  ptx::tc_fence_before();
  __syncthreads();
  run_event(rg, ep, x_img, w_img, chunks, tmem_base, ctrl, nullptr);
  const int row = (quad & 1) * 32 + lane;
  float g[kHiCols / 8][8];
  for (int c0 = cg * 8; c0 < N; c0 += 8 * (kWarps / 4)) {
    acc_take8(t_lane, 0, N, c0, g[c0 / 32]);
    if (quad >= 2)
      for (int j = 0; j < 8; ++j) s_xch[row * kHiCols + c0 + j] = g[c0 / 32][j];
  }
  ptx::tc_fence_before();
  __syncthreads();
  if (quad < 2)
    for (int c0 = cg * 8; c0 < N; c0 += 8 * (kWarps / 4))
      for (int j = 0; j < 8; ++j) C[row * N + c0 + j] = g[c0 / 32][j] + s_xch[row * kHiCols + c0 + j];
  ptx::tc_fence_before();
  __syncthreads();
  if (warp == 2) ptx::tmem_dealloc<kTmemCols>(tmem_base);
}
}

int selftest_umma(const float* A, const float* W, int N, int K, int passes, float* C, cudaStream_t s) {
  (void)passes;
  if (N % 8 != 0 || N < 8 || N > kHiCols || K % kChunkK != 0 || K <= 0)
    return fail(T2_ERR_INVALID, "selftest_umma: N in {8..80 step 8}, K %% 64 == 0");
  const int chunks = K / kChunkK;
  uint8_t *ximg = nullptr, *wimg = nullptr; DecoderCtrl* ctrl = nullptr;
  T2_CUDA(cudaMalloc((void**)&ximg, (size_t)chunks * kXChunkBytes));
  T2_CUDA(cudaMalloc((void**)&wimg, (size_t)chunks * N * 256));
  T2_CUDA(cudaMalloc((void**)&ctrl, sizeof(DecoderCtrl)));
  T2_CUDA(cudaMemsetAsync(ctrl, 0, sizeof(DecoderCtrl), s));
  EventPlan ep; memset(&ep, 0, sizeof(ep));
  ep.ncons = 1; ep.n[0] = N; ep.nrows = N; ep.col0 = 0; ep.w_bytes = N * 256; ep.w_off = 0; ep.chunks = chunks;
  rows_to_image_kernel<<<dim3(chunks, 1), 256, 0, s>>>(A, K, kRows, K, 0, ximg, 0);
  T2_LAUNCH_CHECK();
  pack_rows_image_kernel<<<chunks, 256, 0, s>>>(W, N, K, wimg);
  T2_LAUNCH_CHECK();
  const size_t smem = (size_t)kStages * kStageBytes + 16 * 8 + 16 + (size_t)kRows * kHiCols * 4 + 64;
  T2_CUDA(cudaFuncSetAttribute(selftest_kernel, cudaFuncAttributeMaxDynamicSharedMemorySize, (int)smem));
  selftest_kernel<<<1, kThreads, smem, s>>>(ximg, wimg, ep, chunks, C, N, ctrl);
  T2_LAUNCH_CHECK();
  T2_CUDA(cudaStreamSynchronize(s));
  cudaFree(ximg); cudaFree(wimg); cudaFree(ctrl);
  return T2_OK;
}


#endif

namespace {
constexpr int kBwdTileB = 80, kBwdTileE = 64;

__global__ void pack_bwd_wimg_kernel(const float* __restrict__ w0, int cols0, const float* __restrict__ w1, int cols1,
                                     const BwdCta* __restrict__ plans, uint8_t* __restrict__ wimg) {
  const BwdCta& pc = plans[blockIdx.y];
  const int j = blockIdx.x;
  if (j >= pc.nchunks) return;
  const int n = pc.ep.nrows;
  __half* hi = reinterpret_cast<__half*>(wimg + pc.ep.w_off + (size_t)j * pc.ep.w_bytes);
  __half* lo = hi + n * kChunkK;
  const int n0 = (pc.chunk0 + j) * kChunkK;
  for (int i = threadIdx.x; i < n * kChunkK; i += blockDim.x) {
    const int k = i / n, r = i - k * n;
    const int col = pc.col0 + r;
    const float v = col < cols0 ? w0[(long)(n0 + k) * cols0 + col] : w1[(long)(n0 + k) * cols1 + (col - cols0)];
    __half h, l;
    split_fp16(v, h, l);
    const uint32_t e = img_elem_offset(r, k);
    hi[e] = h; lo[e] = l;
  }
}

__global__ void __launch_bounds__(kThreads, 1)
bwd_gemm_kernel(const uint8_t* __restrict__ x_img, const uint8_t* __restrict__ w_img, const BwdCta* __restrict__ plans,
                const float* __restrict__ inv_scale, float* __restrict__ P, int ldp, DecoderCtrl* ctrl) {
  extern __shared__ __align__(1024) uint8_t smem_raw[];
  const int tid = threadIdx.x, warp = tid >> 5, lane = tid & 31;
  const BwdCta pc = plans[blockIdx.x];
  uint8_t* sp = smem_raw;
  Ring rg;
  rg.stage0 = sp; sp += kStages * kStageBytes;
  uint64_t* bars = reinterpret_cast<uint64_t*>(sp); sp += 16 * sizeof(uint64_t);
  rg.full = bars; rg.empty = bars + kStages; rg.acc = bars + 2 * kStages;
  uint32_t* tmem_slot = reinterpret_cast<uint32_t*>(sp); sp += 16;
  float* s_xch = reinterpret_cast<float*>(sp);
  rg.p_stage = rg.p_phase = rg.c_stage = rg.c_phase = rg.acc_phase = 0;
  rg.pol_x = ptx::policy_evict_last(); rg.pol_w = ptx::policy_evict_first();
  rg.cs = 1; rg.rank = 0; rg.pre = 0; rg.ns = kStages;
  if (tid == 0) {
    for (int s = 0; s < kStages; ++s) { ptx::mbar_init(&rg.full[s], 1); ptx::mbar_init(&rg.empty[s], 1); }
    ptx::mbar_init(rg.acc, 1);
    ptx::fence_barrier_init();
  }
  if (warp == 2) ptx::tmem_alloc<kTmemCols>(tmem_slot);
  ptx::tc_fence_before();
  __syncthreads();
  ptx::tc_fence_after();
  const uint32_t tmem_base = *tmem_slot;
  const int quad = warp & 3, cg = warp >> 2;
  const uint32_t t_lane = tmem_base + ((uint32_t)(quad * 32) << 16);
  for (int c = cg * 40; c < cg * 40 + 40; c += 8) ptx::tmem_zero8(t_lane + c);
  ptx::tmem_wait_st();
  ptx::tc_fence_before();
  __syncthreads();
  run_event(rg, pc.ep, x_img + (size_t)pc.chunk0 * kXChunkBytes, w_img, pc.nchunks, tmem_base, ctrl, nullptr);
  const int N = pc.ep.nrows;
  const int row = (quad & 1) * 32 + lane;
  float g[kHiCols / 32 + 1][8];
  for (int c0 = cg * 8; c0 < N; c0 += 8 * (kWarps / 4)) {
    acc_take8(t_lane, 0, N, c0, g[c0 / 32]);
    if (quad >= 2)
      for (int j = 0; j < 8; ++j) s_xch[row * kHiCols + c0 + j] = g[c0 / 32][j];
  }
  ptx::tc_fence_before();
  __syncthreads();
  if (quad < 2) {
    const float sc = inv_scale[row];
    float* out = P + ((size_t)pc.split * kRows + row) * ldp + pc.col0;
    for (int c0 = cg * 8; c0 < N; c0 += 8 * (kWarps / 4)) {
      float4 v0, v1;
      v0.x = (g[c0 / 32][0] + s_xch[row * kHiCols + c0 + 0]) * sc; v0.y = (g[c0 / 32][1] + s_xch[row * kHiCols + c0 + 1]) * sc;
      v0.z = (g[c0 / 32][2] + s_xch[row * kHiCols + c0 + 2]) * sc; v0.w = (g[c0 / 32][3] + s_xch[row * kHiCols + c0 + 3]) * sc;
      v1.x = (g[c0 / 32][4] + s_xch[row * kHiCols + c0 + 4]) * sc; v1.y = (g[c0 / 32][5] + s_xch[row * kHiCols + c0 + 5]) * sc;
      v1.z = (g[c0 / 32][6] + s_xch[row * kHiCols + c0 + 6]) * sc; v1.w = (g[c0 / 32][7] + s_xch[row * kHiCols + c0 + 7]) * sc;
      *reinterpret_cast<float4*>(out + c0) = v0;
      *reinterpret_cast<float4*>(out + c0 + 4) = v1;
    }
  }
  ptx::tc_fence_before();
  __syncthreads();
  if (warp == 2) ptx::tmem_dealloc<kTmemCols>(tmem_base);
}

size_t bwd_gemm_smem() { return (size_t)kStages * kStageBytes + 16 * 8 + 16 + (size_t)kRows * kHiCols * 4 + 64; }
}

int bwd_gemm_ctas(int which) { return which == 0 ? (2560 / kBwdTileB) * kBwdGemmSplit : (1792 / kBwdTileE) * kBwdGemmSplit; }

int bwd_gemm_prepare(T2Model* m, cudaStream_t s) {
  PersistentPack* pk = (PersistentPack*)m->pk;
  if (!pk) return fail(T2_ERR_INVALID, "backward GEMM: model has no persistent pack");
  for (int which = 0; which < 2; ++which) {
    const int tile = which == 0 ? kBwdTileB : kBwdTileE;
    const int cols = which == 0 ? 2560 : 1792;
    const int ntile = cols / tile, ncta = ntile * kBwdGemmSplit;
    const int chunks = 4 * kARnn / kChunkK;
    const uint32_t w_bytes = (uint32_t)(2 * tile * kChunkK * 2);
    if (!pk->bwd_plans[which]) {
      std::vector<BwdCta> plans(ncta);
      for (int t = 0; t < ntile; ++t)
        for (int sp = 0; sp < kBwdGemmSplit; ++sp) {
          BwdCta& c = plans[t * kBwdGemmSplit + sp];
          memset(&c, 0, sizeof(c));
          c.chunk0 = sp * chunks / kBwdGemmSplit; c.nchunks = (sp + 1) * chunks / kBwdGemmSplit - c.chunk0;
          c.col0 = t * tile; c.split = sp;
          c.ep.nrows = tile; c.ep.col0 = 0; c.ep.ncons = 1; c.ep.n[0] = tile; c.ep.w_bytes = w_bytes; c.ep.chunks = c.nchunks;
          c.ep.w_off = (uint32_t)(((size_t)t * chunks + c.chunk0) * w_bytes);
        }
      T2_CUDA(cudaMalloc((void**)&pk->bwd_plans[which], sizeof(BwdCta) * ncta));
      T2_CUDA(cudaMemcpyAsync(pk->bwd_plans[which], plans.data(), sizeof(BwdCta) * ncta, cudaMemcpyHostToDevice, s));
      T2_CUDA(cudaStreamSynchronize(s));
      T2_CUDA(cudaMalloc((void**)&pk->bwd_wimg[which], (size_t)ntile * chunks * w_bytes));
    }
    const float* w0 = m->w[which == 0 ? W_DRNN_WIH : W_ARNN_WIH];
    const float* w1 = m->w[which == 0 ? W_DRNN_WHH : W_ARNN_WHH];
    const int cols0 = which == 0 ? kARnn + kEnc : kPre + kEnc;
    pack_bwd_wimg_kernel<<<dim3(chunks / kBwdGemmSplit, ncta), 256, 0, s>>>(w0, cols0, w1, kARnn, pk->bwd_plans[which], pk->bwd_wimg[which]);
    T2_LAUNCH_CHECK();
  }
  return T2_OK;
}

int bwd_gemm_run(T2Model* m, int which, const uint8_t* x_img, const float* inv_scale, float* P, int ldp, DecoderCtrl* ctrl,
                 cudaStream_t s) {
  PersistentPack* pk = (PersistentPack*)m->pk;
  const size_t smem = bwd_gemm_smem();
  static bool attr_set = false;
  if (!attr_set) {
    T2_CUDA(cudaFuncSetAttribute(bwd_gemm_kernel, cudaFuncAttributeMaxDynamicSharedMemorySize, (int)smem));
    attr_set = true;
  }
  bwd_gemm_kernel<<<bwd_gemm_ctas(which), kThreads, smem, s>>>(x_img, pk->bwd_wimg[which], pk->bwd_plans[which], inv_scale, P, ldp, ctrl);
  T2_LAUNCH_CHECK();
  return T2_OK;
}

}
```

### tacotron2_b200/csrc/umma.cuh

```cuda
#pragma once
#include <cuda_fp16.h>
#include <stdint.h>

namespace t2 {
namespace ptx {

__device__ __forceinline__ uint32_t smem_u32(const void* p) {
  return static_cast<uint32_t>(__cvta_generic_to_shared(p));
}

__device__ __forceinline__ void mbar_init(uint64_t* bar, uint32_t count) {
  asm volatile("mbarrier.init.shared::cta.b64 [%0], %1;" ::"r"(smem_u32(bar)), "r"(count));
}
__device__ __forceinline__ void fence_barrier_init() {
  asm volatile("fence.mbarrier_init.release.cluster;" ::: "memory");
}
__device__ __forceinline__ void mbar_arrive_expect_tx(uint64_t* bar, uint32_t bytes) {
  asm volatile("mbarrier.arrive.expect_tx.shared::cta.b64 _, [%0], %1;" ::"r"(smem_u32(bar)), "r"(bytes)
               : "memory");
}
__device__ __forceinline__ void mbar_arrive(uint64_t* bar) {
  asm volatile("mbarrier.arrive.shared::cta.b64 _, [%0];" ::"r"(smem_u32(bar)) : "memory");
}
__device__ __forceinline__ bool mbar_try_wait(uint64_t* bar, uint32_t parity) {
  uint32_t ok;
  asm volatile(
      "{\n\t.reg .pred p;\n\t"
      "mbarrier.try_wait.parity.shared::cta.b64 p, [%1], %2;\n\t"
      "selp.u32 %0, 1, 0, p;\n\t}"
      : "=r"(ok)
      : "r"(smem_u32(bar)), "r"(parity)
      : "memory");
  return ok != 0;
}

__device__ __forceinline__ void fence_proxy_async() { asm volatile("fence.proxy.async;" ::: "memory"); }
__device__ __forceinline__ void tc_fence_before() { asm volatile("tcgen05.fence::before_thread_sync;" ::: "memory"); }
__device__ __forceinline__ void tc_fence_after() { asm volatile("tcgen05.fence::after_thread_sync;" ::: "memory"); }

__device__ __forceinline__ void bulk_g2s(void* dst_smem, const void* src_gmem, uint32_t bytes, uint64_t* bar) {
  asm volatile(
      "cp.async.bulk.shared::cluster.global.mbarrier::complete_tx::bytes [%0], [%1], %2, [%3];" ::"r"(
          smem_u32(dst_smem)),
      "l"(src_gmem), "r"(bytes), "r"(smem_u32(bar))
      : "memory");
}

__device__ __forceinline__ uint64_t policy_evict_last() {
  uint64_t pol;
  asm volatile("createpolicy.fractional.L2::evict_last.b64 %0, 1.0;" : "=l"(pol));
  return pol;
}
__device__ __forceinline__ uint64_t policy_evict_first() {
  uint64_t pol;
  asm volatile("createpolicy.fractional.L2::evict_first.b64 %0, 1.0;" : "=l"(pol));
  return pol;
}
__device__ __forceinline__ void bulk_g2s_hint(void* dst_smem, const void* src_gmem, uint32_t bytes, uint64_t* bar,
                                              uint64_t policy) {
  asm volatile(
      "cp.async.bulk.shared::cluster.global.mbarrier::complete_tx::bytes.L2::cache_hint [%0], [%1], %2, [%3], %4;" ::"r"(
          smem_u32(dst_smem)),
      "l"(src_gmem), "r"(bytes), "r"(smem_u32(bar)), "l"(policy)
      : "memory");
}
__device__ __forceinline__ void bulk_g2s_mc_hint(void* dst_smem, const void* src_gmem, uint32_t bytes, uint64_t* bar,
                                                 uint16_t cta_mask, uint64_t policy) {
  asm volatile(
      "cp.async.bulk.shared::cluster.global.mbarrier::complete_tx::bytes.multicast::cluster.L2::cache_hint "
      "[%0], [%1], %2, [%3], %4, %5;" ::"r"(smem_u32(dst_smem)),
      "l"(src_gmem), "r"(bytes), "r"(smem_u32(bar)), "h"(cta_mask), "l"(policy)
      : "memory");
}
__device__ __forceinline__ uint32_t cluster_ctarank() {
  uint32_t r;
  asm volatile("mov.u32 %0, %%cluster_ctarank;" : "=r"(r));
  return r;
}
__device__ __forceinline__ void cluster_sync_all() {
  asm volatile("barrier.cluster.arrive.release.aligned;" ::: "memory");
  asm volatile("barrier.cluster.wait.acquire.aligned;" ::: "memory");
}
__device__ __forceinline__ float4 ldg_f4_hint(const float* p, uint64_t policy) {
  float4 v;
  asm volatile("ld.global.nc.L1::no_allocate.L2::cache_hint.v4.f32 {%0,%1,%2,%3}, [%4], %5;"
               : "=f"(v.x), "=f"(v.y), "=f"(v.z), "=f"(v.w)
               : "l"(p), "l"(policy));
  return v;
}

template <int kCols>
__device__ __forceinline__ void tmem_alloc(uint32_t* dst_smem) {
  asm volatile("tcgen05.alloc.cta_group::1.sync.aligned.shared::cta.b32 [%0], %1;" ::"r"(smem_u32(dst_smem)),
               "n"(kCols)
               : "memory");
  asm volatile("tcgen05.relinquish_alloc_permit.cta_group::1.sync.aligned;" ::: "memory");
}
template <int kCols>
__device__ __forceinline__ void tmem_dealloc(uint32_t taddr) {
  asm volatile("tcgen05.dealloc.cta_group::1.sync.aligned.b32 %0, %1;" ::"r"(taddr), "n"(kCols) : "memory");
}

__device__ __forceinline__ void umma_f16(uint32_t d_tmem, uint64_t a_desc, uint64_t b_desc, uint32_t idesc,
                                         uint32_t accumulate) {
  asm volatile(
      "{\n\t.reg .pred p;\n\t"
      "setp.ne.b32 p, %4, 0;\n\t"
      "tcgen05.mma.cta_group::1.kind::f16 [%0], %1, %2, %3, p;\n\t}" ::"r"(d_tmem),
      "l"(a_desc), "l"(b_desc), "r"(idesc), "r"(accumulate)
      : "memory");
}
__device__ __forceinline__ void umma_commit(uint64_t* bar) {
  asm volatile("tcgen05.commit.cta_group::1.mbarrier::arrive::one.shared::cluster.b64 [%0];" ::"r"(smem_u32(bar))
               : "memory");
}

__device__ __forceinline__ void umma_commit_mc(uint64_t* bar, uint16_t cta_mask) {
  asm volatile(
      "tcgen05.commit.cta_group::1.mbarrier::arrive::one.shared::cluster.multicast::cluster.b64 [%0], %1;" ::"r"(
          smem_u32(bar)),
      "h"(cta_mask)
      : "memory");
}

__device__ __forceinline__ void tmem_ld8(uint32_t taddr, float* v) {
  uint32_t r[8];
  asm volatile("tcgen05.ld.sync.aligned.32x32b.x8.b32 {%0,%1,%2,%3,%4,%5,%6,%7}, [%8];"
               : "=r"(r[0]), "=r"(r[1]), "=r"(r[2]), "=r"(r[3]), "=r"(r[4]), "=r"(r[5]), "=r"(r[6]), "=r"(r[7])
               : "r"(taddr));
  asm volatile("tcgen05.wait::ld.sync.aligned;" ::: "memory");
#pragma unroll
  for (int i = 0; i < 8; ++i) v[i] = __uint_as_float(r[i]);
}

__device__ __forceinline__ void tmem_ld8_issue(uint32_t taddr, uint32_t (&r)[8]) {
  asm volatile("tcgen05.ld.sync.aligned.32x32b.x8.b32 {%0,%1,%2,%3,%4,%5,%6,%7}, [%8];"
               : "=r"(r[0]), "=r"(r[1]), "=r"(r[2]), "=r"(r[3]), "=r"(r[4]), "=r"(r[5]), "=r"(r[6]), "=r"(r[7])
               : "r"(taddr));
}
__device__ __forceinline__ void tmem_ld8_wait(uint32_t (&r)[8]) {
  asm volatile("tcgen05.wait::ld.sync.aligned;"
               : "+r"(r[0]), "+r"(r[1]), "+r"(r[2]), "+r"(r[3]), "+r"(r[4]), "+r"(r[5]), "+r"(r[6]), "+r"(r[7])::"memory");
}

__device__ __forceinline__ void tmem_zero8(uint32_t taddr) {
  const uint32_t z = 0u;
  asm volatile("tcgen05.st.sync.aligned.32x32b.x8.b32 [%0], {%1,%1,%1,%1,%1,%1,%1,%1};" ::"r"(taddr), "r"(z) : "memory");
}
__device__ __forceinline__ void tmem_wait_st() { asm volatile("tcgen05.wait::st.sync.aligned;" ::: "memory"); }

__device__ __forceinline__ uint64_t make_smem_desc(uint32_t smem_addr, uint32_t lbo, uint32_t sbo) {
  uint64_t d = 0;
  d |= (uint64_t)((smem_addr & 0x3FFFFu) >> 4);
  d |= (uint64_t)((lbo >> 4) & 0x3FFFu) << 16;
  d |= (uint64_t)((sbo >> 4) & 0x3FFFu) << 32;
  d |= (uint64_t)1 << 46;
  return d;
}
__device__ __forceinline__ uint64_t make_sw128_desc(uint32_t smem_addr) {
  uint64_t d = 0;
  d |= (uint64_t)((smem_addr & 0x3FFFFu) >> 4);
  d |= (uint64_t)1 << 16;
  d |= (uint64_t)(1024u >> 4) << 32;
  d |= (uint64_t)1 << 46;
  d |= (uint64_t)2 << 61;
  return d;
}
__device__ __forceinline__ uint32_t make_idesc_f16(uint32_t M, uint32_t N) {
  return (1u << 4) | ((N >> 3) << 17) | ((M >> 4) << 24);
}
__device__ __forceinline__ uint32_t make_idesc_f16_m64(uint32_t N) { return make_idesc_f16(64, N); }

}

constexpr int kChunkK = 64;
__host__ __device__ inline uint32_t img_elem_offset(int r, int k) {
  return (uint32_t)((r >> 3) * 512 + (r & 7) * 64 + ((((k >> 3) ^ (r & 7)) & 7) * 8) + (k & 7));
}
__device__ __forceinline__ void split_fp16(float x, __half& hi, __half& lo) {
  hi = __float2half_rn(x);
  lo = __float2half_rn(x - __half2float(hi));
}

}
```

Baseline: 1.160 million.

## Offload prenet x1/x2 tail to a dedicated 4-CTA cluster with DSMEM exchange

Adds four extra tail CTAs in one cluster that recompute the dh-projection for the prenet columns, apply the prenet layer-1 ReLU and dropout, broadcast the x1 image to each other through distributed shared memory, and run the prenet layer-2 GEMM from shared-memory-resident weights. This removes the grid-wide x1/x2 events from the main 128 CTAs, shrinks the projection CTA set, and drops the optional cluster and hierarchical barrier modes. In exchange, the tail duplicates some GEMM work, the launch must have 132 co-resident CTAs with cluster size 4, and new per-chunk x2 counters add synchronization complexity.

```diff
diff --git a/tacotron2_b200/_engine.py b/tacotron2_b200/_engine.py
--- a/tacotron2_b200/_engine.py
+++ b/tacotron2_b200/_engine.py
@@ -319,7 +319,8 @@
         out = (C.c_int64 * 72)()
         _capi.check(_capi.lib().t2_decoder_profile(C.byref(a), out))
         names = ["E0 x2->att gemm", "E0 epilogue(ah)", "B1", "E1 ah->dec/att/q gemm", "B2", "attention", "B3",
-                 "E2 ctx gemm", "E2 epilogue(dh)", "B4", "E3 dh gemm", "E3 epilogue(mel/x1)", "B5", "E4 x1 gemm+epi", "B6",
+                 "E2 ctx gemm", "E2 epilogue(dh)", "B4", "E3 dh gemm", "E3 epilogue(mel/gate)", "gate arrive", "(unused)",
+                 "wait x2 chunk 0",
                  "att:im2col", "att:mma", "att:energies", "att:softmax", "att:context"]
         return {names[i]: [int(out[s * 24 + i]) for s in range(3)] for i in range(len(names))}
 
diff --git a/tacotron2_b200/csrc/decoder.h b/tacotron2_b200/csrc/decoder.h
--- a/tacotron2_b200/csrc/decoder.h
+++ b/tacotron2_b200/csrc/decoder.h
@@ -14,8 +14,8 @@
   int pad2_[2];
   int done[kMaxBatch];
   long long prof[3][24];
-  unsigned int x1_count; int pad3_[31];
-  unsigned int x2_count; int pad4_[31];
+  unsigned int gate_count; int pad3_[31];
+  unsigned int x2_count[16]; int pad4_[16];
   unsigned int ah_count[16]; int pad5_[16];
   unsigned int dh_count[16]; int pad6_[16];
 };
diff --git a/tacotron2_b200/csrc/decoder_persistent.cu b/tacotron2_b200/csrc/decoder_persistent.cu
--- a/tacotron2_b200/csrc/decoder_persistent.cu
+++ b/tacotron2_b200/csrc/decoder_persistent.cu
@@ -12,6 +12,9 @@
 namespace {
 
 constexpr int kG = 128;
+constexpr int kTail = 4;
+constexpr int kGrid = kG + kTail;
+constexpr int kCluster = kTail;
 constexpr int kThreads = 512;
 constexpr int kWarps = kThreads / 32;
 constexpr int kStages = 4;
@@ -26,9 +29,21 @@
 constexpr int kWStageMax = 2 * kHiCols * kChunkK * 2;
 constexpr int kStageBytes = kXChunkBytes + kWStageMax;
 constexpr int kNumEvents = 5;
-constexpr int kPCols = 344;
-constexpr int kQCta0 = 0, kQCtas = 16, kX2Cta0 = 16, kX2Ctas = 32, kPCta0 = 48, kPCtas = 43;
+constexpr int kPCols = kMel + 1 + kPre;
+constexpr int kQCta0 = 0, kQCtas = 16, kPCta0 = 48, kPCtas = 11;
 constexpr int kWeffBytes = kAtt * kChunkK * 2 * 2;
+constexpr int kRowTab = 64;
+constexpr int kTailN = 64;
+constexpr int kColX1 = 0, kColX2 = 2 * kTailN;
+constexpr int kTailStages = 4;
+constexpr int kTailStageBytes = kXChunkBytes + 2 * kTailN * kChunkK * 2;
+constexpr int kW2Bytes = (kPre / kChunkK) * 2 * kTailN * kChunkK * 2;
+constexpr int kTailPrefixBytes = (kTailStages * kTailStageBytes + kW2Bytes + 2 * 64 * 8 + kTailN * 4 + 1023) & ~1023;
+static_assert(2 * kTailStageBytes >= 4 * (2 * 64 * kChunkK * 2) && kTailStages >= 3 &&
+              kTailStageBytes >= 64 * (kTailN + 1) * 4, "tail ring stages 0-1: x1 image, stage 2: epilogue exchange");
+__host__ __device__ constexpr int smem_prefix_bytes(int nstages) {
+  return nstages * kStageBytes + kWeffBytes > kTailPrefixBytes ? nstages * kStageBytes + kWeffBytes : kTailPrefixBytes;
+}
 constexpr int kXchStride = 33;
 constexpr unsigned long long kWatchdogCycles = 1ull << 32;
 
@@ -107,8 +122,8 @@
 
 __global__ void pack_consumer_kernel(const float* __restrict__ src, int ld, int kcol0,
                                      const int32_t* __restrict__ rows_tab, const CtaPlan* __restrict__ plans,
-                                     int ev, int cons, uint8_t* __restrict__ wimg) {
-  const int cta = blockIdx.y, chunk = blockIdx.x;
+                                     int ev, int cons, int cta0, uint8_t* __restrict__ wimg) {
+  const int cta = cta0 + blockIdx.y, chunk = blockIdx.x;
   const EventPlan& ep = plans[cta].ev[ev];
   if (cons >= ep.ncons) return;
   const int n = ep.n[cons];
@@ -117,7 +132,7 @@
   __half* img = reinterpret_cast<__half*>(wimg + ep.w_off + (size_t)chunk * ep.w_bytes);
   for (int i = threadIdx.x; i < n * 64; i += blockDim.x) {
     const int r = i >> 6, k = i & 63;
-    const int srow = rows_tab[cta * 32 + r];
+    const int srow = rows_tab[cta * kRowTab + r];
     const float v = srow >= 0 ? src[(long)srow * ld + kcol0 + chunk * 64 + k] : 0.f;
     __half h, l;
     split_fp16(v, h, l);
@@ -180,29 +195,10 @@
   asm volatile("fence.acq_rel.gpu;" ::: "memory");
 }
 
-__device__ __forceinline__ void grid_barrier(DecoderCtrl* ctrl, unsigned int& target, uint32_t cs, uint32_t rank) {
+__device__ __forceinline__ void grid_barrier(DecoderCtrl* ctrl, unsigned int& target) {
   ptx::fence_proxy_async();
-  if (cs > 1) {
-    __threadfence();
-    ptx::cluster_sync_all();
-    target += gridDim.x / cs;
-    if (rank == 0 && threadIdx.x == 0) {
-      asm volatile("red.release.gpu.global.add.u32 [%0], 1;" ::"l"(&ctrl->bar_count) : "memory");
-      const unsigned long long t0 = clock64();
-      while (true) {
-        unsigned int c;
-        asm volatile("ld.acquire.gpu.global.u32 %0, [%1];" : "=r"(c) : "l"(&ctrl->bar_count) : "memory");
-        if ((int)(c - target) >= 0) break;
-        if (clock64() - t0 > kWatchdogCycles) watchdog_trap(ctrl, 100);
-      }
-      __threadfence();
-    }
-    ptx::cluster_sync_all();
-    ptx::fence_proxy_async();
-    return;
-  }
-  __syncthreads();
-  target += gridDim.x;
+  __syncthreads();
+  target += kG;
   if (threadIdx.x == 0) {
     arrive_release(&ctrl->bar_count);
     poll_acquire(&ctrl->bar_count, target, ctrl, 100);
@@ -214,7 +210,7 @@
 __device__ __forceinline__ void grid_arrive(DecoderCtrl* ctrl, unsigned int& target) {
   ptx::fence_proxy_async();
   __syncthreads();
-  target += gridDim.x;
+  target += kG;
   if (threadIdx.x == 0) {
     arrive_release(&ctrl->bar_count);
   }
@@ -269,7 +265,8 @@
 
 struct Ring {
   uint8_t* stage0;
-  __device__ __forceinline__ uint8_t* stage(uint32_t s) const { return stage0 + s * kStageBytes; }
+  uint32_t sb;
+  __device__ __forceinline__ uint8_t* stage(uint32_t s) const { return stage0 + s * sb; }
   uint64_t* full;
   uint64_t* empty;
   uint64_t* acc;
@@ -277,7 +274,6 @@
   uint32_t c_stage, c_phase;
   uint32_t acc_phase;
   uint64_t pol_x, pol_w;
-  uint32_t cs, rank;
   uint32_t pre;
   uint32_t ns;
 };
@@ -334,13 +330,7 @@
           asm volatile("fence.acq_rel.gpu;" ::: "memory");
           ptx::fence_proxy_async();
         }
-        if (rg.cs == 1) {
-          ptx::bulk_g2s_hint(st, x_img + (size_t)i * kXChunkBytes, kXChunkBytes, &rg.full[rg.p_stage], rg.pol_x);
-        } else {
-          const uint32_t slice = kXChunkBytes / rg.cs;
-          ptx::bulk_g2s_mc_hint(st + rg.rank * slice, x_img + (size_t)i * kXChunkBytes + rg.rank * slice, slice,
-                                &rg.full[rg.p_stage], (uint16_t)((1u << rg.cs) - 1u), rg.pol_x);
-        }
+        ptx::bulk_g2s_hint(st, x_img + (size_t)i * kXChunkBytes, kXChunkBytes, &rg.full[rg.p_stage], rg.pol_x);
         if (++rg.p_stage == rg.ns) { rg.p_stage = 0; rg.p_phase ^= 1; }
       }
       rg.pre = 0;
@@ -362,8 +352,7 @@
           const uint64_t b = ptx::make_sw128_desc(ws + kk * 32);
           ptx::umma_f16(d, a, b, idesc, 1u);
         }
-        if (rg.cs == 1) ptx::umma_commit(&rg.empty[rg.c_stage]);
-        else ptx::umma_commit_mc(&rg.empty[rg.c_stage], (uint16_t)((1u << rg.cs) - 1u));
+        ptx::umma_commit(&rg.empty[rg.c_stage]);
         if (++rg.c_stage == rg.ns) { rg.c_stage = 0; rg.c_phase ^= 1; }
       }
       ptx::umma_commit(rg.acc);
@@ -421,12 +410,12 @@
   float l2_pin_frac;
   const float* memory; const float* pm; const int32_t* mem_len;
   const uint8_t* prenet_keep; const uint8_t* att_keep; const uint8_t* dec_keep;
-  uint8_t* x2_img; uint8_t* ah_img; uint8_t* ctx_img; uint8_t* dh_img; uint8_t* x1_img;
+  uint8_t* x2_img; uint8_t* ah_img; uint8_t* ctx_img; uint8_t* dh_img;
   const uint8_t* teacher_x2_img;
   float* q;
   float* mel; float* gate; float* align; int32_t* mel_lengths; int32_t* n_steps;
   DecoderCtrl* ctrl;
-  int B, T, cap, infer, training, cluster, hier_barrier;
+  int B, T, cap, infer, training;
   int nstages;
   int chunk_ready;
   int b0, Btot;
@@ -451,14 +440,21 @@
   extern __shared__ __align__(1024) uint8_t smem_raw[];
   const int tid = threadIdx.x, warp = tid >> 5, lane = tid & 31;
   const int cta = blockIdx.x;
+  const bool tail = cta >= kG;
   const int T = p.T, TP = T + kLocK - 1;
   const int ntiles = (T + 127) >> 7;
 
   uint8_t* sp = smem_raw;
   Ring rg;
-  rg.ns = (uint32_t)p.nstages;
-  rg.stage0 = sp; sp += p.nstages * kStageBytes;
-  uint8_t* s_weff = sp; sp += kWeffBytes;
+  rg.ns = (uint32_t)(tail ? kTailStages : p.nstages);
+  rg.stage0 = sp;
+  rg.sb = tail ? kTailStageBytes : kStageBytes;
+  uint8_t* s_weff = sp + p.nstages * kStageBytes;
+  uint8_t* s_w2 = rg.stage0 + kTailStages * kTailStageBytes;
+  uint8_t* s_keep = s_w2 + kW2Bytes;
+  float* s_bias_x1 = reinterpret_cast<float*>(s_keep + 2 * kRows * 8);
+  uint8_t* x1_smem = rg.stage0;
+  sp += smem_prefix_bytes(p.nstages);
   uint64_t* bars = reinterpret_cast<uint64_t*>(sp); sp += 16 * sizeof(uint64_t);
   rg.full = bars; rg.empty = bars + kMaxStages; rg.acc = bars + 2 * kMaxStages;
   uint32_t* tmem_slot = reinterpret_cast<uint32_t*>(sp); sp += 16;
@@ -469,7 +465,6 @@
   float* s_v = reinterpret_cast<float*>(sp); sp += kAtt * 4;
   float* s_q = reinterpret_cast<float*>(sp); sp += kAtt * 4;
   float* s_red = reinterpret_cast<float*>(sp); sp += 32 * 4;
-  uint32_t* s_mask = reinterpret_cast<uint32_t*>(sp); sp += kRows * 4;
   float* s_bias_p = reinterpret_cast<float*>(sp); sp += 8 * 4;
   long long* s_prof = reinterpret_cast<long long*>(sp); sp += 24 * 8;
   float* s_pad0 = reinterpret_cast<float*>(sp); sp += ((TP + 3) & ~3) * 4;
@@ -480,18 +475,24 @@
   (void)s_red;
 
   rg.p_stage = rg.p_phase = rg.c_stage = rg.c_phase = rg.acc_phase = 0;
-  rg.cs = p.cluster; rg.rank = p.cluster > 1 ? ptx::cluster_ctarank() : 0;
   rg.pre = 0;
 
+  const CtaPlan& plan = p.plans[cta];
   if (tid == 0) {
-    for (int s = 0; s < p.nstages; ++s) { ptx::mbar_init(&rg.full[s], 1); ptx::mbar_init(&rg.empty[s], rg.cs); }
+    for (uint32_t s = 0; s < rg.ns; ++s) { ptx::mbar_init(&rg.full[s], 1); ptx::mbar_init(&rg.empty[s], 1); }
     ptx::mbar_init(rg.acc, 1);
     ptx::fence_barrier_init();
   }
   if (warp == 2) ptx::tmem_alloc<kTmemCols>(tmem_slot);
-  for (int i = tid; i < 32; i += kThreads) { s_bias_a[i] = p.bias_a[cta * 32 + i]; s_bias_d[i] = p.bias_d[cta * 32 + i]; }
-  for (int i = tid; i < kWeffBytes / 16; i += kThreads)
-    reinterpret_cast<uint4*>(s_weff)[i] = reinterpret_cast<const uint4*>(p.weff_img)[i];
+  if (!tail) {
+    for (int i = tid; i < 32; i += kThreads) { s_bias_a[i] = p.bias_a[cta * 32 + i]; s_bias_d[i] = p.bias_d[cta * 32 + i]; }
+    for (int i = tid; i < kWeffBytes / 16; i += kThreads)
+      reinterpret_cast<uint4*>(s_weff)[i] = reinterpret_cast<const uint4*>(p.weff_img)[i];
+  } else if (p.infer) {
+    const uint4* w2 = reinterpret_cast<const uint4*>(p.wimg + plan.ev[4].w_off);
+    for (int i = tid; i < kW2Bytes / 16; i += kThreads) reinterpret_cast<uint4*>(s_w2)[i] = w2[i];
+    for (int i = tid; i < kTailN; i += kThreads) s_bias_x1[i] = p.bias_p[kMel + 1 + (cta - kG) * kTailN + i];
+  }
   {
     uint64_t pol;
     asm volatile("createpolicy.fractional.L2::evict_last.L2::evict_first.b64 %0, %1;" : "=l"(pol) : "f"(p.l2_pin_frac));
@@ -504,14 +505,12 @@
   ptx::fence_proxy_async();
   ptx::tc_fence_before();
   __syncthreads();
-  if (p.cluster > 1) ptx::cluster_sync_all();
+  ptx::cluster_sync_all();
   ptx::tc_fence_after();
   const uint32_t tmem_base = *tmem_slot;
 
-  const CtaPlan& plan = p.plans[cta];
   DecoderCtrl* ctrl = p.ctrl;
   unsigned int bar_target = 0;
-  const uint32_t bar_cs = p.hier_barrier ? rg.cs : 1;
   const int quad = warp & 3, cg = warp >> 2;
   const int row = (quad & 1) * 32 + lane;
   const bool is_lo = quad >= 2;
@@ -519,10 +518,12 @@
   const uint32_t t_lane = tmem_base + ((uint32_t)(quad * 32) << 16);
   float c_att[2] = {0.f, 0.f}, c_dec[2] = {0.f, 0.f};
   const bool has_q = cta >= kQCta0 && cta < kQCta0 + kQCtas;
-  const bool has_x2 = cta >= kX2Cta0 && cta < kX2Cta0 + kX2Ctas;
   const bool has_p = cta >= kPCta0 && cta < kPCta0 + kPCtas;
   const int halfk = (kLocK - 1) / 2;
-  for (int c = cg * 40; c < cg * 40 + 40; c += 8) ptx::tmem_zero8(t_lane + c);
+  {
+    const int zc = tail ? (kColX2 + 2 * kTailN) / 4 : 40;
+    for (int c = cg * zc; c < cg * zc + zc; c += 8) ptx::tmem_zero8(t_lane + c);
+  }
   ptx::tmem_wait_st();
   ptx::tc_fence_before();
   __syncthreads();
@@ -550,32 +551,136 @@
     }                                                                                    \
   } while (0)
 
-  auto x2_epilogue = [&]() {
-    float g[8];
-    if (cg == 0) acc_take8(t_lane, kColS, kNS, 0, g);
-    if (cg == 0 && is_lo) {
-#pragma unroll
-      for (int i = 0; i < 8; ++i) s_xch[row * kXchStride + i] = g[i];
+  int t = 0;
+  if (tail && p.infer) {
+    const int k = cta - kG;
+    const EventPlan& ev2 = plan.ev[2];
+    const EventPlan& ev3 = plan.ev[3];
+    const uint32_t x1_local = ptx::smem_u32(x1_smem);
+    float* s_xt = reinterpret_cast<float*>(rg.stage0 + 2 * kTailStageBytes);
+    auto take16 = [&](int base, float (&g)[16]) {
+      acc_take8(t_lane, base, kTailN, cg * 16, g);
+      acc_take8(t_lane, base, kTailN, cg * 16 + 8, g + 8);
+      if (is_lo) {
+#pragma unroll
+        for (int j = 0; j < 16; ++j) s_xt[row * (kTailN + 1) + cg * 16 + j] = g[j];
+      }
+      ptx::tc_fence_before();
+      __syncthreads();
+      if (!is_lo) {
+#pragma unroll
+        for (int j = 0; j < 16; ++j) g[j] += s_xt[row * (kTailN + 1) + cg * 16 + j];
+      }
+    };
+    if (tid == 0) prefetch_weights(rg, ev2, p.wimg, ctrl);
+    for (; t < p.cap; ++t) {
+      const bool last = t + 1 == p.cap;
+      if (!last) {
+        const int r = tid >> 3, grp = tid & 7, col0 = k * kTailN + grp * 8;
+        if (r < p.B) {
+#pragma unroll
+          for (int site = 0; site < 2; ++site) {
+            uint32_t bits = 0;
+            if (p.prenet_keep) {
+              const uint8_t* kp = p.prenet_keep + ((long)(t + 1) * 2 + site) * p.Btot * kPre + (long)(p.b0 + r) * kPre + col0;
+              for (int j = 0; j < 8; ++j) bits |= (kp[j] != 0 ? 1u : 0u) << j;
+            } else {
+              bits = philox_keep8(p.seed, (t + 1) * 4 + site, (uint64_t)(p.b0 + r) * kPre + col0, 0.5f);
+            }
+            s_keep[site * kRows * 8 + r * 8 + grp] = (uint8_t)bits;
+          }
+        }
+      }
+      bar_target += kG * (p.chunk_ready ? 2u : 3u);
+      grid_wait(ctrl, bar_target);
+      run_event(rg, ev2, p.ctx_img, p.wimg, 8, tmem_base, ctrl, &ev3);
+      if (!p.chunk_ready) { bar_target += kG; grid_wait(ctrl, bar_target); }
+      run_event(rg, ev3, p.dh_img, p.wimg, 16, tmem_base, ctrl, nullptr,
+                p.chunk_ready ? ctrl->dh_count : nullptr, 8u * (unsigned int)(t + 1));
+      ptx::cluster_arrive();
+      float g[16];
+      take16(kColX1, g);
+      uint4 xh[2], xl[2];
+      if (!is_lo) {
+#pragma unroll
+        for (int h = 0; h < 2; ++h) {
+          const uint32_t bits = s_keep[row * 8 + 2 * cg + h];
+          __align__(16) __half hh[8];
+          __align__(16) __half ll[8];
+#pragma unroll
+          for (int j = 0; j < 8; ++j) {
+            float r = fmaxf(g[8 * h + j] + s_bias_x1[cg * 16 + 8 * h + j], 0.f);
+            if (!last) r = ((bits >> j) & 1u) ? r * 2.f : 0.f;
+            if (row >= p.B) r = 0.f;
+            split_fp16(r, hh[j], ll[j]);
+          }
+          xh[h] = *reinterpret_cast<const uint4*>(hh);
+          xl[h] = *reinterpret_cast<const uint4*>(ll);
+        }
+      }
+      bool stop = last;
+      stop |= wait_counter(&ctrl->gate_count, (unsigned int)(t + 1), s_flag, ctrl, 102);
+      ptx::cluster_wait();
+      if (!is_lo) {
+#pragma unroll
+        for (int h = 0; h < 2; ++h) {
+          const uint32_t off = (uint32_t)k * kXChunkBytes + img_elem_offset(row, cg * 16 + 8 * h) * 2;
+#pragma unroll
+          for (int r = 0; r < kTail; ++r) {
+            const uint32_t dst = ptx::mapa(x1_local + off, (uint32_t)r);
+            ptx::st_cluster_v4(dst, xh[h]);
+            ptx::st_cluster_v4(dst + kRows * kChunkK * 2, xl[h]);
+          }
+        }
+      }
+      ptx::fence_proxy_async_cluster();
+      ptx::cluster_arrive();
+      ptx::cluster_wait();
+      ptx::fence_proxy_async();
+      if (!last) {
+        if (warp == 1) {
+          if (lane == 0) {
+            ptx::tc_fence_after();
+            const uint32_t idesc = ptx::make_idesc_f16(128, 2u * kTailN);
+#pragma unroll
+            for (int i = 0; i < kPre / kChunkK; ++i) {
+              const uint32_t xs = x1_local + i * kXChunkBytes, ws = ptx::smem_u32(s_w2) + i * plan.ev[4].w_bytes;
+#pragma unroll
+              for (int kk = 0; kk < kChunkK / 16; ++kk)
+                ptx::umma_f16(tmem_base + kColX2, ptx::make_sw128_desc(xs + kk * 32), ptx::make_sw128_desc(ws + kk * 32),
+                              idesc, 1u);
+            }
+            ptx::umma_commit(rg.acc);
+          }
+          __syncwarp();
+        }
+        mbar_wait(rg.acc, rg.acc_phase, ctrl, 207);
+        rg.acc_phase ^= 1;
+        ptx::tc_fence_after();
+        take16(kColX2, g);
+        if (erow) {
+#pragma unroll
+          for (int h = 0; h < 2; ++h) {
+            const uint32_t bits = s_keep[kRows * 8 + row * 8 + 2 * cg + h];
+            float r[8];
+#pragma unroll
+            for (int j = 0; j < 8; ++j) r[j] = ((bits >> j) & 1u) ? fmaxf(g[8 * h + j], 0.f) * 2.f : 0.f;
+#pragma unroll
+            for (int j = 0; j < 8; j += 2)
+              store_split2(p.x2_img, row, k * kTailN + cg * 16 + 8 * h + j, r[j], r[j + 1]);
+          }
+        }
+      }
+      signal_counter(&ctrl->x2_count[k], 1u + (stop ? kStopFlag : 0u));
+      if (stop) { ++t; break; }
+      if (tid == 0) prefetch_weights(rg, ev2, p.wimg, ctrl);
     }
-    ptx::tc_fence_before();
-    __syncthreads();
-    if (cg == 0 && erow) {
-      const int col0 = (cta - kX2Cta0) * 8;
-      float r[8];
-      const uint32_t bits = s_mask[row];
-#pragma unroll
-      for (int j = 0; j < 8; ++j)
-        r[j] = ((bits >> j) & 1u) ? fmaxf(g[j] + s_xch[row * kXchStride + j], 0.f) * 2.f : 0.f;
-#pragma unroll
-      for (int j = 0; j < 8; j += 2) store_split2(p.x2_img, row, col0 + j, r[j], r[j + 1]);
-    }
-  };
-
-  int t = 0;
-  for (; t < p.cap; ++t) {
+  }
+  for (; !tail && t < p.cap; ++t) {
     {
       const uint8_t* x2 = p.infer ? p.x2_img : p.teacher_x2_img + (size_t)t * 4 * kXChunkBytes;
-      run_event(rg, plan.ev[0], x2, p.wimg, 4, tmem_base, ctrl, &plan.ev[1]);
+      run_event(rg, plan.ev[0], x2, p.wimg, 4, tmem_base, ctrl, &plan.ev[1],
+                (p.infer && t > 0) ? ctrl->x2_count : nullptr, (unsigned int)t);
       T2_PROF(0);
       float g[8];
       T2_TAKE_GATES(kColA, kNA, g);
@@ -605,33 +710,10 @@
       }
       T2_PROF(1);
       if (p.chunk_ready) signal_counter(&ctrl->ah_count[cta >> 3], 1u);
-      else grid_barrier(ctrl, bar_target, bar_cs, rg.rank);
+      else grid_barrier(ctrl, bar_target);
       T2_PROF(2);
     }
     {
-      if (p.infer && is_lo && cg == 0 && row < p.B && t + 1 < p.cap && (has_p || has_x2)) {
-        uint32_t bits = 0;
-        if (has_x2) {
-          const int col0 = (cta - kX2Cta0) * 8;
-          if (p.prenet_keep) {
-            const uint8_t* kp = p.prenet_keep + ((long)(t + 1) * 2 + 1) * p.Btot * kPre + (long)(p.b0 + row) * kPre + col0;
-            for (int j = 0; j < 8; ++j) bits |= (kp[j] != 0 ? 1u : 0u) << j;
-          } else {
-            bits = philox_keep8(p.seed, (t + 1) * 4 + 1, (uint64_t)(p.b0 + row) * kPre + col0, 0.5f);
-          }
-        } else {
-          const int pc0 = (cta - kPCta0) * 8;
-          for (int j = 0; j < 8; ++j) {
-            const int col = pc0 + j - (kMel + 1);
-            if (col < 0 || col >= kPre) continue;
-            const long idx = (long)(p.b0 + row) * kPre + col;
-            const bool keep = p.prenet_keep ? p.prenet_keep[((long)(t + 1) * 2 + 0) * p.Btot * kPre + idx] != 0
-                                            : philox_keep(p.seed, (t + 1) * 4 + 0, idx, 0.5f);
-            bits |= (keep ? 1u : 0u) << j;
-          }
-        }
-        s_mask[row] = bits;
-      }
       run_event(rg, plan.ev[1], p.ah_img, p.wimg, 16, tmem_base, ctrl, nullptr,
                 p.chunk_ready ? ctrl->ah_count : nullptr, 8u * (unsigned int)(t + 1));
       if (has_q) {
@@ -839,7 +921,7 @@
       T2_PROF(19);
     }
     T2_PROF(5);
-    grid_barrier(ctrl, bar_target, bar_cs, rg.rank);
+    grid_barrier(ctrl, bar_target);
     T2_PROF(6);
     {
       run_event(rg, plan.ev[2], p.ctx_img, p.wimg, 8, tmem_base, ctrl, &plan.ev[3]);
@@ -872,12 +954,12 @@
       }
       T2_PROF(8);
       if (p.chunk_ready) signal_counter(&ctrl->dh_count[cta >> 3], 1u);
-      else grid_barrier(ctrl, bar_target, bar_cs, rg.rank);
+      else grid_barrier(ctrl, bar_target);
       T2_PROF(9);
     }
     {
       run_event(rg, plan.ev[3], p.dh_img, p.wimg, 16, tmem_base, ctrl,
-                (!p.infer && t + 1 < p.cap) ? &plan.ev[0] : nullptr,
+                t + 1 < p.cap ? &plan.ev[0] : nullptr,
                 p.chunk_ready ? ctrl->dh_count : nullptr, 8u * (unsigned int)(t + 1));
       T2_PROF(10);
       if (tid == 0) *s_live = 0;
@@ -906,18 +988,6 @@
               }
               if (!done) atomicAdd(s_live, 1);
             }
-          } else if (pc < kMel + 1 + kPre) {
-            const int col = pc - (kMel + 1);
-            float r = fmaxf(v, 0.f);
-            if (p.infer && t + 1 < p.cap) r = ((s_mask[row] >> j) & 1u) ? r * 2.f : 0.f;
-            if (p.infer) {
-              __half h, l;
-              split_fp16(r, h, l);
-              __half* hi = reinterpret_cast<__half*>(p.x1_img + (size_t)(col >> 6) * kXChunkBytes);
-              __half* lo = hi + kRows * kChunkK;
-              const uint32_t e = img_elem_offset(row, col & 63);
-              hi[e] = h; lo[e] = l;
-            }
           }
         }
       }
@@ -927,19 +997,22 @@
       T2_PROF(11);
       if (!p.infer) continue;
       bool stop = t + 1 == p.cap;
-      if (has_p) signal_counter(&ctrl->x1_count, 1u + ((gate_cta && *s_live == 0) ? kStopFlag : 0u));
-      if (has_x2) {
-        stop |= wait_counter(&ctrl->x1_count, (unsigned int)(kPCtas * (t + 1)), s_flag, ctrl, 102);
-        if (!stop) {
-          run_event(rg, plan.ev[4], p.x1_img, p.wimg, 4, tmem_base, ctrl, nullptr);
-          x2_epilogue();
-        }
-        signal_counter(&ctrl->x2_count, 1u + (stop ? kStopFlag : 0u));
-      }
+      if (gate_cta) signal_counter(&ctrl->gate_count, 1u + (*s_live == 0 ? kStopFlag : 0u));
       T2_PROF(12);
-      stop |= wait_counter(&ctrl->x2_count, (unsigned int)(kX2Ctas * (t + 1)), s_flag, ctrl, 103);
+      stop |= wait_counter(&ctrl->x2_count[0], (unsigned int)(t + 1), s_flag, ctrl, 103);
       T2_PROF(14);
-      if (stop) { ++t; break; }
+      if (stop) {
+        if (tid == 0) {
+          uint32_t st = rg.p_stage, ph = rg.p_phase;
+          for (uint32_t i = 0; i < rg.pre; ++i) {
+            ptx::bulk_g2s_hint(rg.stage(st), p.x2_img + (size_t)i * kXChunkBytes, kXChunkBytes, &rg.full[st], rg.pol_x);
+            mbar_wait(&rg.full[st], ph, ctrl, 208);
+            if (++st == rg.ns) { st = 0; ph ^= 1; }
+          }
+        }
+        ++t;
+        break;
+      }
     }
   }
   if (prof_slot >= 0 && tid == 0)
@@ -951,15 +1024,8 @@
       if (!p.infer || !__ldcg(&ctrl->done[b])) p.mel_lengths[b] = ns;
     if (tid == 0) atomicMax(p.n_steps, ns);
   }
-  if (p.cluster > 1) {
-    if (tid == 0)
-      for (int s = 0; s < p.nstages; ++s) {
-        mbar_wait(&rg.empty[rg.p_stage], rg.p_phase ^ 1, ctrl, 204);
-        if (++rg.p_stage == rg.ns) { rg.p_stage = 0; rg.p_phase ^= 1; }
-      }
-    __syncthreads();
-    ptx::cluster_sync_all();
-  }
+  __syncthreads();
+  ptx::cluster_sync_all();
   ptx::tc_fence_before();
   __syncthreads();
   if (warp == 2) ptx::tmem_dealloc<kTmemCols>(tmem_base);
@@ -971,8 +1037,8 @@
   const int TP = T + kLocK - 1;
   const int ntiles = (T + 127) / 128;
   const size_t xch = (size_t)kRows * kXchStride * 4, att = (size_t)5 * ntiles * 128 * 4;
-  return (size_t)nstages * kStageBytes + kWeffBytes + 16 * 8 + 16 + 16 + 2 * 32 * 4 + kAtt * 4 + kAtt * 4 + 32 * 4 +
-         kRows * 4 + 32 + 24 * 8 + 2 * (size_t)((TP + 3) & ~3) * 4 + (xch > att ? xch : att) + 1024;
+  return (size_t)smem_prefix_bytes(nstages) + 16 * 8 + 16 + 16 + 2 * 32 * 4 + kAtt * 4 + kAtt * 4 + 32 * 4 +
+         32 + 24 * 8 + 2 * (size_t)((TP + 3) & ~3) * 4 + (xch > att ? xch : att) + 1024;
 }
 constexpr size_t kSmemLimit = 227 * 1024;
 static int persistent_stages(int T) {
@@ -985,13 +1051,13 @@
 
 size_t persistent_ws_bytes(int B, int T, int cap) {
   (void)B; (void)T;
-  return (size_t)(4 + 16 + 8 + 16 + 4) * kXChunkBytes + (size_t)kRows * kAtt * 4 + 1024 +
+  return (size_t)(4 + 16 + 8 + 16) * kXChunkBytes + (size_t)kRows * kAtt * 4 + 1024 +
          (size_t)cap * 4 * kXChunkBytes;
 }
 
 bool persistent_supported(const T2Model* m, const T2DecoderArgs* a) {
   if (!m->pk) return false;
-  if (m->sm_count < kG) return false;
+  if (m->sm_count < kGrid) return false;
   if (persistent_smem_bytes(a->T_enc, 4) > kSmemLimit) return false;
   return true;
 }
@@ -1000,11 +1066,10 @@
   PersistentPack* pk = (PersistentPack*)m->pk;
   if (!pk) { pk = new PersistentPack(); m->pk = pk; }
   const int kdc = kDRnn + kEnc;
-  std::vector<CtaPlan> plans(kG);
+  std::vector<CtaPlan> plans(kGrid);
   size_t off = 0;
-  for (int c = 0; c < kG; ++c) {
-    const bool hq = c >= kQCta0 && c < kQCta0 + kQCtas, hx = c >= kX2Cta0 && c < kX2Cta0 + kX2Ctas,
-               hp = c >= kPCta0 && c < kPCta0 + kPCtas;
+  for (int c = 0; c < kGrid; ++c) {
+    const bool hq = c >= kQCta0 && c < kQCta0 + kQCtas, hp = c >= kPCta0 && c < kPCta0 + kPCtas;
     CtaPlan& pl = plans[c];
     memset(&pl, 0, sizeof(pl));
     auto set = [&](int ev, int chunks, int col0, std::initializer_list<int> ns) {
@@ -1016,22 +1081,29 @@
       e.chunks = chunks;
       off += (size_t)chunks * e.w_bytes;
     };
+    if (c >= kG) {
+      pl.ev[0].w_off = pl.ev[1].w_off = (uint32_t)off;
+      set(2, 8, kColX1, {kTailN});
+      set(3, 16, kColX1, {kTailN});
+      set(4, kPre / kChunkK, kColX2, {kTailN});
+      continue;
+    }
     set(0, 4, kColA, {32});
     if (hq) set(1, 16, kColA, {32, 32, 16}); else set(1, 16, kColA, {32, 32});
     if (hp) set(2, 8, kColA, {32, 32, 16}); else set(2, 8, kColA, {32, 32});
     if (hp) set(3, 16, kColD, {32, 16}); else set(3, 16, kColD, {32});
-    if (hx) set(4, 4, kColS, {16}); else { pl.ev[4].w_off = (uint32_t)off; }
+    pl.ev[4].w_off = (uint32_t)off;
   }
   if (off >= (size_t)4 << 30) return fail(T2_ERR_INVALID, "W image too large");
   if (!pk->wimg) {
     pk->wimg_bytes = off + 1024;
     T2_CUDA(cudaMalloc((void**)&pk->wimg, pk->wimg_bytes));
-    T2_CUDA(cudaMalloc((void**)&pk->plans, sizeof(CtaPlan) * kG));
+    T2_CUDA(cudaMalloc((void**)&pk->plans, sizeof(CtaPlan) * kGrid));
     T2_CUDA(cudaMalloc((void**)&pk->wp_all, (size_t)kPCols * kdc * 4));
     T2_CUDA(cudaMalloc((void**)&pk->bias_p, (size_t)kPCols * 4));
     T2_CUDA(cudaMalloc((void**)&pk->bias_a, (size_t)kG * 32 * 4));
     T2_CUDA(cudaMalloc((void**)&pk->bias_d, (size_t)kG * 32 * 4));
-    T2_CUDA(cudaMalloc((void**)&pk->rows, (size_t)4 * kG * 32 * 4));
+    T2_CUDA(cudaMalloc((void**)&pk->rows, (size_t)4 * kGrid * kRowTab * 4));
     T2_CUDA(cudaMalloc((void**)&pk->weff, (size_t)kAtt * kChunkK * 4));
     T2_CUDA(cudaMalloc((void**)&pk->weff_img, (size_t)kWeffBytes));
   }
@@ -1039,7 +1111,7 @@
   T2_LAUNCH_CHECK();
   pack_rows_image_kernel<<<1, 256, 0, s>>>(pk->weff, kAtt, kChunkK, pk->weff_img);
   T2_LAUNCH_CHECK();
-  T2_CUDA(cudaMemcpyAsync(pk->plans, plans.data(), sizeof(CtaPlan) * kG, cudaMemcpyHostToDevice, s));
+  T2_CUDA(cudaMemcpyAsync(pk->plans, plans.data(), sizeof(CtaPlan) * kGrid, cudaMemcpyHostToDevice, s));
   T2_CUDA(cudaStreamSynchronize(s));
   T2_CUDA(cudaMemsetAsync(pk->wp_all, 0, (size_t)kPCols * kdc * 4, s));
   T2_CUDA(cudaMemsetAsync(pk->bias_p, 0, (size_t)kPCols * 4, s));
@@ -1052,19 +1124,29 @@
   T2_LAUNCH_CHECK();
   pack_lstm_bias_kernel<<<(kG * 32 + 255) / 256, 256, 0, s>>>(m->drnn_b, pk->bias_d);
   T2_LAUNCH_CHECK();
-  std::vector<int32_t> rows((size_t)4 * kG * 32, -1);
+  std::vector<int32_t> rows((size_t)4 * kGrid * kRowTab, -1);
   for (int c = 0; c < kG; ++c) {
-    for (int col = 0; col < 32; ++col) rows[(0 * kG + c) * 32 + col] = (col & 3) * 1024 + c * 8 + (col >> 2);
-    if (c >= kQCta0 && c < kQCta0 + kQCtas) for (int j = 0; j < 8; ++j) rows[(1 * kG + c) * 32 + j] = (c - kQCta0) * 8 + j;
-    if (c >= kPCta0 && c < kPCta0 + kPCtas) for (int j = 0; j < 8; ++j) rows[(2 * kG + c) * 32 + j] = (c - kPCta0) * 8 + j;
-    if (c >= kX2Cta0 && c < kX2Cta0 + kX2Ctas) for (int j = 0; j < 8; ++j) rows[(3 * kG + c) * 32 + j] = (c - kX2Cta0) * 8 + j;
-  }
+    for (int col = 0; col < 32; ++col) rows[(0 * kGrid + c) * kRowTab + col] = (col & 3) * 1024 + c * 8 + (col >> 2);
+    if (c >= kQCta0 && c < kQCta0 + kQCtas)
+      for (int j = 0; j < 8; ++j) rows[(1 * kGrid + c) * kRowTab + j] = (c - kQCta0) * 8 + j;
+    if (c >= kPCta0 && c < kPCta0 + kPCtas)
+      for (int j = 0; j < 8; ++j) {
+        const int pc = (c - kPCta0) * 8 + j;
+        rows[(2 * kGrid + c) * kRowTab + j] = pc <= kMel ? pc : -1;
+      }
+  }
+  for (int c = kG; c < kGrid; ++c)
+    for (int j = 0; j < kTailN; ++j) {
+      rows[(2 * kGrid + c) * kRowTab + j] = kMel + 1 + (c - kG) * kTailN + j;
+      rows[(3 * kGrid + c) * kRowTab + j] = (c - kG) * kTailN + j;
+    }
   T2_CUDA(cudaMemcpyAsync(pk->rows, rows.data(), rows.size() * 4, cudaMemcpyHostToDevice, s));
   T2_CUDA(cudaStreamSynchronize(s));
-  const int32_t* r_lstm = pk->rows; const int32_t* r_q = pk->rows + kG * 32;
-  const int32_t* r_p = pk->rows + 2 * kG * 32; const int32_t* r_x2 = pk->rows + 3 * kG * 32;
-  auto pack = [&](const float* src, int ld, int kcol0, int chunks, const int32_t* rt, int ev, int cons) -> int {
-    pack_consumer_kernel<<<dim3(chunks, kG), 256, 0, s>>>(src, ld, kcol0, rt, pk->plans, ev, cons, pk->wimg);
+  const int32_t* r_lstm = pk->rows; const int32_t* r_q = pk->rows + kGrid * kRowTab;
+  const int32_t* r_p = pk->rows + 2 * kGrid * kRowTab; const int32_t* r_x2 = pk->rows + 3 * kGrid * kRowTab;
+  auto pack = [&](const float* src, int ld, int kcol0, int chunks, const int32_t* rt, int ev, int cons, int cta0 = 0,
+                  int n = kG) -> int {
+    pack_consumer_kernel<<<dim3(chunks, n), 256, 0, s>>>(src, ld, kcol0, rt, pk->plans, ev, cons, cta0, pk->wimg);
     T2_LAUNCH_CHECK();
     return T2_OK;
   };
@@ -1077,7 +1159,9 @@
   T2_TRY(pack(pk->wp_all, kdc, kDRnn, 8, r_p, 2, 2));
   T2_TRY(pack(m->w[W_DRNN_WHH], kDRnn, 0, 16, r_lstm, 3, 0));
   T2_TRY(pack(pk->wp_all, kdc, 0, 16, r_p, 3, 1));
-  T2_TRY(pack(m->w[W_PRENET1], kPre, 0, 4, r_x2, 4, 0));
+  T2_TRY(pack(pk->wp_all, kdc, kDRnn, 8, r_p, 2, 0, kG, kTail));
+  T2_TRY(pack(pk->wp_all, kdc, 0, 16, r_p, 3, 0, kG, kTail));
+  T2_TRY(pack(m->w[W_PRENET1], kPre, 0, kPre / kChunkK, r_x2, 4, 0, kG, kTail));
   return T2_OK;
 }
 
@@ -1108,7 +1192,7 @@
   DecoderWs w;
   T2_TRY(decoder_ws_carve(a, &w));
   T2_CUDA(cudaMemsetAsync(w.ctrl, 0, sizeof(DecoderCtrl), s));
-  T2_CUDA(cudaMemsetAsync(w.persistent, 0, (size_t)(4 + 16 + 8 + 16 + 4) * kXChunkBytes + (size_t)kRows * kAtt * 4, s));
+  T2_CUDA(cudaMemsetAsync(w.persistent, 0, (size_t)(4 + 16 + 8 + 16) * kXChunkBytes + (size_t)kRows * kAtt * 4, s));
   {
     GemmArgs g;
     g.seg[0] = {a->memory + (size_t)b0 * T * kEnc, kEnc, m->w[W_ATT_MEMORY], kEnc, kEnc};
@@ -1122,7 +1206,6 @@
   p.ah_img = img; img += 16 * kXChunkBytes;
   p.ctx_img = img; img += 8 * kXChunkBytes;
   p.dh_img = img; img += 16 * kXChunkBytes;
-  p.x1_img = img; img += 4 * kXChunkBytes;
   p.q = (float*)img;
   p.plans = pk->plans; p.wimg = pk->wimg; p.bias_a = pk->bias_a; p.bias_d = pk->bias_d; p.bias_p = pk->bias_p;
   p.weff_img = pk->weff_img; p.w_v = m->w[W_ATT_V];
@@ -1160,53 +1243,34 @@
   }
   p.nstages = persistent_stages(T);
   {
-  }
-  {
     const char* e = getenv("T2_CHUNK_READY");
     p.chunk_ready = (e && !strcmp(e, "0")) ? 0 : 1;
   }
   const size_t smem = persistent_smem_bytes(T, p.nstages);
   T2_CUDA(cudaFuncSetAttribute(decoder_persistent_kernel, cudaFuncAttributeMaxDynamicSharedMemorySize, (int)smem));
-  T2_CUDA(cudaFuncSetAttribute(decoder_persistent_kernel, cudaFuncAttributeNonPortableClusterSizeAllowed, 1));
-  int want = 1;
-  {
-    const char* e = getenv("T2_CLUSTER");
-    if (e) want = atoi(e);
-    if (want != 1 && want != 2 && want != 4 && want != 8) want = 1;
-  }
-  {
-    p.hier_barrier = 0;
-  }
   cudaLaunchConfig_t cfg;
   memset(&cfg, 0, sizeof(cfg));
-  cfg.gridDim = dim3(kG); cfg.blockDim = dim3(kThreads); cfg.dynamicSmemBytes = smem; cfg.stream = s;
+  cfg.gridDim = dim3(kGrid); cfg.blockDim = dim3(kThreads); cfg.dynamicSmemBytes = smem; cfg.stream = s;
   cudaLaunchAttribute attrs[2];
-  for (p.cluster = want; p.cluster > 1; p.cluster >>= 1) {
-    attrs[0].id = cudaLaunchAttributeClusterDimension;
-    attrs[0].val.clusterDim.x = p.cluster; attrs[0].val.clusterDim.y = 1; attrs[0].val.clusterDim.z = 1;
-    cfg.attrs = attrs; cfg.numAttrs = 1;
-    int max_clusters = 0;
-    if (cudaOccupancyMaxActiveClusters(&max_clusters, decoder_persistent_kernel, &cfg) == cudaSuccess &&
-        max_clusters * p.cluster >= kG)
-      break;
-    (void)cudaGetLastError();
-  }
-  int na = 0;
-  if (p.cluster > 1) {
-    attrs[na].id = cudaLaunchAttributeClusterDimension;
-    attrs[na].val.clusterDim.x = p.cluster; attrs[na].val.clusterDim.y = 1; attrs[na].val.clusterDim.z = 1; ++na;
-  }
-  attrs[na].id = cudaLaunchAttributeCooperative; attrs[na].val.cooperative = 1; ++na;
-  cfg.attrs = attrs; cfg.numAttrs = na;
+  attrs[0].id = cudaLaunchAttributeClusterDimension;
+  attrs[0].val.clusterDim.x = kCluster; attrs[0].val.clusterDim.y = 1; attrs[0].val.clusterDim.z = 1;
+  cfg.attrs = attrs; cfg.numAttrs = 1;
+  int max_clusters = 0;
+  T2_CUDA(cudaOccupancyMaxActiveClusters(&max_clusters, decoder_persistent_kernel, &cfg));
+  if (max_clusters * kCluster < kGrid)
+    return fail(T2_ERR_UNSUPPORTED, "persistent decoder: only %d clusters of %d co-resident, %d needed", max_clusters,
+                kCluster, kGrid / kCluster);
+  attrs[1].id = cudaLaunchAttributeCooperative; attrs[1].val.cooperative = 1;
+  cfg.numAttrs = 2;
   cudaError_t le = cudaLaunchKernelEx(&cfg, decoder_persistent_kernel, p);
-  if (le != cudaSuccess && p.cluster > 1) {
+  if (le != cudaSuccess) {
     (void)cudaGetLastError();
     cfg.numAttrs = 1;
     le = cudaLaunchKernelEx(&cfg, decoder_persistent_kernel, p);
   }
   if (le != cudaSuccess) return fail(T2_ERR_CUDA, "persistent decoder launch failed: %s", cudaGetErrorString(le));
-  if (getenv("T2_VERBOSE")) fprintf(stderr, "[t2b200] persistent decoder: B=%d T_enc=%d cap=%d cluster=%d stages=%d chunk_ready=%d smem=%zu\n",
-                                    B, T, cap, p.cluster, p.nstages, p.chunk_ready, smem);
+  if (getenv("T2_VERBOSE")) fprintf(stderr, "[t2b200] persistent decoder: B=%d T_enc=%d cap=%d clusters=%d/%d stages=%d chunk_ready=%d smem=%zu\n",
+                                    B, T, cap, kGrid / kCluster, max_clusters, p.nstages, p.chunk_ready, smem);
   g_launch_count++;
   return T2_OK;
 }
@@ -1221,13 +1285,14 @@
   uint8_t* sp = smem_raw;
   Ring rg;
   rg.stage0 = sp; sp += kStages * kStageBytes;
+  rg.sb = kStageBytes;
   uint64_t* bars = reinterpret_cast<uint64_t*>(sp); sp += 16 * sizeof(uint64_t);
   rg.full = bars; rg.empty = bars + kStages; rg.acc = bars + 2 * kStages;
   uint32_t* tmem_slot = reinterpret_cast<uint32_t*>(sp); sp += 16;
   float* s_xch = reinterpret_cast<float*>(sp);
   rg.p_stage = rg.p_phase = rg.c_stage = rg.c_phase = rg.acc_phase = 0;
   rg.pol_x = rg.pol_w = ptx::policy_evict_last();
-  rg.cs = 1; rg.rank = 0; rg.pre = 0; rg.ns = kStages;
+  rg.pre = 0; rg.ns = kStages;
   if (tid == 0) {
     for (int s = 0; s < kStages; ++s) { ptx::mbar_init(&rg.full[s], 1); ptx::mbar_init(&rg.empty[s], 1); }
     ptx::mbar_init(rg.acc, 1);
@@ -1326,13 +1391,14 @@
   uint8_t* sp = smem_raw;
   Ring rg;
   rg.stage0 = sp; sp += kStages * kStageBytes;
+  rg.sb = kStageBytes;
   uint64_t* bars = reinterpret_cast<uint64_t*>(sp); sp += 16 * sizeof(uint64_t);
   rg.full = bars; rg.empty = bars + kStages; rg.acc = bars + 2 * kStages;
   uint32_t* tmem_slot = reinterpret_cast<uint32_t*>(sp); sp += 16;
   float* s_xch = reinterpret_cast<float*>(sp);
   rg.p_stage = rg.p_phase = rg.c_stage = rg.c_phase = rg.acc_phase = 0;
   rg.pol_x = ptx::policy_evict_last(); rg.pol_w = ptx::policy_evict_first();
-  rg.cs = 1; rg.rank = 0; rg.pre = 0; rg.ns = kStages;
+  rg.pre = 0; rg.ns = kStages;
   if (tid == 0) {
     for (int s = 0; s < kStages; ++s) { ptx::mbar_init(&rg.full[s], 1); ptx::mbar_init(&rg.empty[s], 1); }
     ptx::mbar_init(rg.acc, 1);
diff --git a/tacotron2_b200/csrc/umma.cuh b/tacotron2_b200/csrc/umma.cuh
--- a/tacotron2_b200/csrc/umma.cuh
+++ b/tacotron2_b200/csrc/umma.cuh
@@ -77,9 +77,23 @@
   asm volatile("mov.u32 %0, %%cluster_ctarank;" : "=r"(r));
   return r;
 }
+__device__ __forceinline__ void cluster_arrive() { asm volatile("barrier.cluster.arrive.release.aligned;" ::: "memory"); }
+__device__ __forceinline__ void cluster_wait() { asm volatile("barrier.cluster.wait.acquire.aligned;" ::: "memory"); }
 __device__ __forceinline__ void cluster_sync_all() {
-  asm volatile("barrier.cluster.arrive.release.aligned;" ::: "memory");
-  asm volatile("barrier.cluster.wait.acquire.aligned;" ::: "memory");
+  cluster_arrive();
+  cluster_wait();
+}
+__device__ __forceinline__ uint32_t mapa(uint32_t smem_addr, uint32_t rank) {
+  uint32_t r;
+  asm volatile("mapa.shared::cluster.u32 %0, %1, %2;" : "=r"(r) : "r"(smem_addr), "r"(rank));
+  return r;
+}
+__device__ __forceinline__ void st_cluster_v4(uint32_t addr, const uint4& v) {
+  asm volatile("st.shared::cluster.v4.u32 [%0], {%1,%2,%3,%4};" ::"r"(addr), "r"(v.x), "r"(v.y), "r"(v.z), "r"(v.w)
+               : "memory");
+}
+__device__ __forceinline__ void fence_proxy_async_cluster() {
+  asm volatile("fence.proxy.async.shared::cluster;" ::: "memory");
 }
 __device__ __forceinline__ float4 ldg_f4_hint(const float* p, uint64_t policy) {
   float4 v;
```

After: 1.126 million, median of 6. -3.0%, worse.
